# Symb0x76/ChineseChessZero

Measured on NVIDIA B200. Metric: self-play moves/sec at 400 playouts, higher is better.
Workload: dtype bf16

## Files before the change

### chinesechesszero_b200/_lib.py

```python
from __future__ import annotations

import ctypes
import os

import numpy as np
import torch

from . import build as _build

BOARD_BYTES = 96
MAX_MOVES = 128
N_ACTIONS = 2086
PLANE_ELEMS = 10710
KEY_WINDOW = 128

FLAG_CHECK, FLAG_NOMOVES, FLAG_INSUFFICIENT, FLAG_FOURFOLD, FLAG_SIXTY = 1, 2, 4, 8, 16
FLAG_TIE_MASK = FLAG_INSUFFICIENT | FLAG_FOURFOLD | FLAG_SIXTY
STATUS_EXPAND_FAILED, STATUS_TREE_DROPPED = 1, 2
STATUS_NODE_OVERFLOW = STATUS_EXPAND_FAILED
ADVANCE_NEW_GAME, ADVANCE_DROP_TREE, ADVANCE_KEEP = -1, -2, -3
CTL_HEAD, CTL_TAIL, CTL_EXPAND_FAILED, CTL_TREES_DROPPED, CTL_MIN_FREE, CTL_WORDS = 0, 1, 2, 3, 4, 8
NODE_BYTES = 24
MAX_CHILDREN = 119
POLICY_PROBS, POLICY_LOGITS = 0, 1
CONV_VARIANT_1CTA, CONV_VARIANT_PAIR, CONV_VARIANT_2PAIRS, CONV_VARIANT_4PAIRS = 1, 2, 2 | 32, 2 | 64

EXPORTS = (
    "ccz_version", "ccz_last_error", "ccz_init", "ccz_action_table", "ccz_set_order_policy", "ccz_get_order_policy",
    "ccz_boards_start",
    "ccz_movegen_encode", "ccz_board_keys_init", "ccz_board_push", "ccz_mcts_pool_init", "ccz_mcts_reset",
    "ccz_mcts_reserve", "ccz_mcts_migrate", "ccz_mcts_select",
    "ccz_mcts_expand_backup", "ccz_mcts_root_visits", "ccz_mcts_advance", "ccz_replay_pack", "ccz_conv3x3_c256", "ccz_conv3x3_plan", "ccz_stem_lookup",
    "ccz_heads_pack",
)


class CczError(RuntimeError):
    pass


class ArenaStruct(ctypes.Structure):

    _fields_ = [
        ("n_games", ctypes.c_int32),
        ("n_pages", ctypes.c_int32),
        ("page_shift", ctypes.c_int32),
        ("max_pages", ctypes.c_int32),
        ("d_nodes", ctypes.c_void_p),
        ("d_links", ctypes.c_void_p),
        ("d_free_ring", ctypes.c_void_p),
        ("d_pool_ctl", ctypes.c_void_p),
        ("d_page_list", ctypes.c_void_p),
        ("d_page_fill", ctypes.c_void_p),
        ("d_n_pages", ctypes.c_void_p),
        ("d_n_pages_new", ctypes.c_void_p),
        ("d_list_sel", ctypes.c_void_p),
        ("d_alloc_page", ctypes.c_void_p),
        ("d_alloc_off", ctypes.c_void_p),
        ("d_root", ctypes.c_void_p),
        ("d_n_nodes", ctypes.c_void_p),
        ("d_status", ctypes.c_void_p),
        ("d_root_boards", ctypes.c_void_p),
        ("d_root_keys", ctypes.c_void_p),
    ]


_lib = None


def library_path() -> str:
    return os.environ.get("CCZ_LIB") or _build.OUT


def load() -> ctypes.CDLL:
    global _lib
    if _lib is not None:
        return _lib
    path = library_path()
    if path == _build.OUT and _build.is_stale():
        try:
            _build.build()
        except Exception as e:
            if not os.path.exists(path):
                raise CczError(f"building {path} failed ({e}); there is no CPU fallback") from e
    if not os.path.exists(path):
        raise CczError(
            f"{path} is missing: run `python -c 'import __graft_entry__ as g; g.build()'` "
            "(nvcc -gencode arch=compute_100a,code=sm_100a); there is no CPU fallback"
        )
    lib = ctypes.CDLL(path)
    vp, i32, f32 = ctypes.c_void_p, ctypes.c_int, ctypes.c_float
    lib.ccz_version.restype = i32
    lib.ccz_last_error.restype = ctypes.c_char_p
    lib.ccz_init.restype = i32
    lib.ccz_action_table.argtypes = [vp, vp, vp]
    lib.ccz_boards_start.argtypes = [vp, i32, vp]
    lib.ccz_set_order_policy.argtypes = [vp]
    lib.ccz_get_order_policy.argtypes = [vp]
    lib.ccz_movegen_encode.argtypes = [vp, i32, vp, vp, vp, vp, vp]
    lib.ccz_board_keys_init.argtypes = [vp, i32, vp, vp]
    lib.ccz_board_push.argtypes = [vp, vp, i32, vp, vp]
    lib.ccz_mcts_pool_init.argtypes = [ctypes.POINTER(ArenaStruct), vp]
    lib.ccz_mcts_reset.argtypes = [ctypes.POINTER(ArenaStruct), vp, vp]
    lib.ccz_mcts_reserve.argtypes = [ctypes.POINTER(ArenaStruct), i32, vp]
    lib.ccz_mcts_migrate.argtypes = [ctypes.POINTER(ArenaStruct), ctypes.POINTER(ArenaStruct), vp]
    lib.ccz_mcts_select.argtypes = [ctypes.POINTER(ArenaStruct), f32, vp, vp, vp]
    lib.ccz_mcts_expand_backup.argtypes = [ctypes.POINTER(ArenaStruct), vp, vp, i32, vp, vp, vp, vp, vp]
    lib.ccz_mcts_root_visits.argtypes = [ctypes.POINTER(ArenaStruct), vp, vp, vp, vp]
    lib.ccz_mcts_advance.argtypes = [ctypes.POINTER(ArenaStruct), vp, vp]
    lib.ccz_replay_pack.argtypes = [vp, vp, vp, vp, vp, i32, vp, vp, vp]
    lib.ccz_conv3x3_c256.argtypes = [vp, vp, vp, vp, vp, i32, i32, vp]
    lib.ccz_stem_lookup.argtypes = [vp, i32, vp, vp, vp, vp]
    lib.ccz_conv3x3_plan.argtypes = [i32, i32, i32, vp]
    lib.ccz_heads_pack.argtypes = [vp, i32, vp, i32, i32, vp]
    for name in EXPORTS:
        if name not in ("ccz_last_error",):
            getattr(lib, name).restype = i32
    _lib = lib
    pinned = os.path.join(os.path.dirname(os.path.abspath(__file__)), "order_policy.json")
    if os.path.exists(pinned):
        import json

        with open(pinned) as f:
            set_order_policy(json.load(f))
    return lib


def check(rc: int, what: str) -> None:
    if rc != 0:
        msg = load().ccz_last_error().decode("utf-8", "replace")
        raise CczError(f"{what} failed ({rc}): {msg}")


def stream_ptr(device=None) -> int:
    return torch.cuda.current_stream(device).cuda_stream


def _ptr(t: torch.Tensor | None) -> int | None:
    if t is None:
        return None
    if not t.is_cuda:
        raise CczError("device tensor expected (the C ABI takes device pointers)")
    if not t.is_contiguous():
        raise CczError("contiguous tensor expected")
    return t.data_ptr()


def host_action_table():
    id_of = np.empty(8100, dtype=np.int16)
    fr = np.empty(N_ACTIONS, dtype=np.uint8)
    to = np.empty(N_ACTIONS, dtype=np.uint8)
    n = load().ccz_action_table(id_of.ctypes.data, fr.ctypes.data, to.ctypes.data)
    if n != N_ACTIONS:
        raise CczError(f"ccz_action_table returned {n}")
    return id_of.reshape(90, 90), fr, to


PIECE_SYMBOLS = (None, "p", "c", "r", "n", "b", "a", "k")
DEFAULT_ORDER_POLICY = {"class_rank": {"p": 1, "c": 0, "r": 0, "n": 0, "b": 0, "a": 0, "k": 0},
                        "from_descending": 1, "to_descending": 1, "capture_mode": 0, "check_king_first": 0}


def set_order_policy(policy: dict | None = None) -> None:
    if policy is None:
        check(load().ccz_set_order_policy(None), "ccz_set_order_policy")
        return
    ranks = [0] * 8
    for sym, r in policy["class_rank"].items():
        ranks[PIECE_SYMBOLS.index(sym)] = int(r)
    raw = bytes(ranks + [int(policy["from_descending"]), int(policy["to_descending"]), int(policy["capture_mode"]),
                        int(policy.get("check_king_first", 0))])
    check(load().ccz_set_order_policy(ctypes.create_string_buffer(raw, 12)), "ccz_set_order_policy")


def get_order_policy() -> dict:
    buf = ctypes.create_string_buffer(12)
    check(load().ccz_get_order_policy(buf), "ccz_get_order_policy")
    b = buf.raw
    return {"class_rank": {PIECE_SYMBOLS[t]: b[t] for t in range(1, 8)}, "from_descending": b[8],
            "to_descending": b[9], "capture_mode": b[10], "check_king_first": b[11]}



def boards_start(n: int, device="cuda") -> torch.Tensor:
    boards = torch.empty((n, BOARD_BYTES), dtype=torch.uint8, device=device)
    with torch.cuda.device(boards.device):
        check(load().ccz_boards_start(_ptr(boards), n, stream_ptr(boards.device)), "ccz_boards_start")
    return boards


def movegen_encode(boards: torch.Tensor, planes: bool = True, out=None):
    n = boards.shape[0]
    dev = boards.device
    _ptr(boards)
    if out is None:
        move_ids = torch.empty((n, MAX_MOVES), dtype=torch.int16, device=dev)
        counts = torch.empty((n,), dtype=torch.int16, device=dev)
        flags = torch.empty((n,), dtype=torch.uint8, device=dev)
        pl = torch.empty((n, 17, 7, 10, 9), dtype=torch.bfloat16, device=dev) if planes else None
    else:
        move_ids, counts, flags, pl = out
    with torch.cuda.device(dev):
        check(
            load().ccz_movegen_encode(_ptr(boards), n, _ptr(move_ids), _ptr(counts), _ptr(flags), _ptr(pl),
                                      stream_ptr(dev)),
            "ccz_movegen_encode",
        )
    return move_ids, counts, flags, pl


def board_keys_init(boards: torch.Tensor) -> torch.Tensor:
    n = boards.shape[0]
    keys = torch.empty((n, KEY_WINDOW), dtype=torch.int64, device=boards.device)
    with torch.cuda.device(boards.device):
        check(load().ccz_board_keys_init(_ptr(boards), n, _ptr(keys), stream_ptr(boards.device)),
              "ccz_board_keys_init")
    return keys


def board_push(boards: torch.Tensor, move_ids: torch.Tensor, keys: torch.Tensor | None = None) -> None:
    n = boards.shape[0]
    if move_ids.dtype != torch.int16 or move_ids.numel() != n:
        raise CczError("move_ids must be int16 [n]")
    with torch.cuda.device(boards.device):
        check(load().ccz_board_push(_ptr(boards), _ptr(move_ids), n, _ptr(keys), stream_ptr(boards.device)),
              "ccz_board_push")


def search_pages(n_playout: int, page_shift: int) -> int:
    runs_per_page = max(1, (1 << page_shift) // MAX_CHILDREN)
    return -(-int(n_playout) // runs_per_page) + 1


class Arena:

    def __init__(self, n_games: int, n_pages: int, page_shift: int = 11, max_pages: int | None = None, device="cuda"):
        self.n_games, self.n_pages, self.page_shift = int(n_games), int(n_pages), int(page_shift)
        if not 7 <= self.page_shift <= 16:
            raise CczError("page_shift must be 7..16")
        if self.n_pages < self.n_games:
            raise CczError("the pool needs at least one page per game")
        if (self.n_pages << self.page_shift) >= 1 << 31:
            raise CczError("pool too large: n_pages << page_shift must stay below 2^31 nodes")
        self.max_pages = int(max_pages) if max_pages is not None else min(self.n_pages, 4096)
        self.device = torch.device(device)
        total = self.n_pages << self.page_shift
        g, z = self.n_games, dict(device=self.device)
        i32 = torch.int32
        self.nodes = torch.empty((total, 4), dtype=i32, **z)
        self.links = torch.empty((total, 2), dtype=i32, **z)
        self.free_ring = torch.zeros(self.n_pages, dtype=i32, **z)
        self.pool_ctl = torch.zeros(CTL_WORDS, dtype=torch.int64, **z)
        self.page_lists = torch.zeros((2, g, self.max_pages), dtype=i32, **z)
        self.page_fill = torch.zeros((g, self.max_pages), dtype=i32, **z)
        self.n_pages_game = torch.zeros(g, dtype=i32, **z)
        self.n_pages_new = torch.zeros(g, dtype=i32, **z)
        self.list_sel = torch.zeros(g, dtype=i32, **z)
        self.alloc_page = torch.zeros(g, dtype=i32, **z)
        self.alloc_off = torch.zeros(g, dtype=i32, **z)
        self.root = torch.zeros(g, dtype=i32, **z)
        self.n_nodes = torch.zeros(g, dtype=i32, **z)
        self.status = torch.zeros(g, dtype=i32, **z)
        self.root_boards = torch.zeros((g, BOARD_BYTES), dtype=torch.uint8, **z)
        self.root_keys = torch.zeros((g, KEY_WINDOW), dtype=torch.int64, **z)
        self._tensors = (self.nodes, self.links, self.free_ring, self.pool_ctl, self.page_lists, self.page_fill,
                         self.n_pages_game, self.n_pages_new, self.list_sel, self.alloc_page, self.alloc_off, self.root,
                         self.n_nodes, self.status, self.root_boards, self.root_keys)
        self.struct = ArenaStruct(self.n_games, self.n_pages, self.page_shift, self.max_pages,
                                  *(t.data_ptr() for t in self._tensors))
        with torch.cuda.device(self.device):
            check(load().ccz_mcts_pool_init(self.ref, stream_ptr(self.device)), "ccz_mcts_pool_init")

    @property
    def ref(self):
        return ctypes.byref(self.struct)

    @property
    def page_nodes(self) -> int:
        return 1 << self.page_shift

    def bytes(self) -> int:
        return sum(t.numel() * t.element_size() for t in self._tensors)

    def pool_stats(self) -> dict:
        c = self.pool_ctl.cpu().numpy()
        free = int(c[CTL_TAIL] - c[CTL_HEAD])
        return {"n_pages": self.n_pages, "page_nodes": self.page_nodes, "free_pages": free,
                "min_free_pages": int(c[CTL_MIN_FREE]), "expand_failed": int(c[CTL_EXPAND_FAILED]),
                "trees_dropped": int(c[CTL_TREES_DROPPED])}

    def node_fields(self, idx: torch.Tensor) -> dict:
        idx = idx.to(torch.int64)
        n, l = self.nodes[idx], self.links[idx]
        word = l[..., 1]
        return {"visits": n[..., 0], "value": n[..., 1].contiguous().view(torch.float32),
                "prior": n[..., 2].contiguous().view(torch.float32), "first_child": n[..., 3], "parent": l[..., 0],
                "move": ((word & 0xFFFF) ^ 0x8000) - 0x8000, "n_child": word >> 16}

    def children(self, node: int) -> dict:
        f = self.node_fields(torch.tensor([node], device=self.device))
        fc, nc = int(f["first_child"][0]), int(f["n_child"][0])
        return self.node_fields(torch.arange(fc, fc + nc, device=self.device))


def mcts_reset(a: Arena, mask: torch.Tensor | None = None) -> None:
    if mask is not None and (mask.dtype != torch.uint8 or mask.numel() != a.n_games):
        raise CczError("mask must be uint8 [n_games]")
    with torch.cuda.device(a.device):
        check(load().ccz_mcts_reset(a.ref, _ptr(mask), stream_ptr(a.device)), "ccz_mcts_reset")


def mcts_select(a: Arena, c_puct: float, leaf_boards: torch.Tensor, leaf_nodes: torch.Tensor) -> None:
    with torch.cuda.device(a.device):
        check(load().ccz_mcts_select(a.ref, float(c_puct), _ptr(leaf_boards), _ptr(leaf_nodes), stream_ptr(a.device)),
              "ccz_mcts_select")


def mcts_expand_backup(a: Arena, leaf_nodes, policy, policy_kind, values, move_ids, counts, flags) -> None:
    if policy.dtype != torch.float32 or values.dtype != torch.float32:
        raise CczError("policy and values must be float32")
    with torch.cuda.device(a.device):
        check(
            load().ccz_mcts_expand_backup(a.ref, _ptr(leaf_nodes), _ptr(policy), int(policy_kind), _ptr(values),
                                          _ptr(move_ids), _ptr(counts), _ptr(flags), stream_ptr(a.device)),
            "ccz_mcts_expand_backup",
        )


def mcts_root_visits(a: Arena, acts, visits, counts) -> None:
    with torch.cuda.device(a.device):
        check(load().ccz_mcts_root_visits(a.ref, _ptr(acts), _ptr(visits), _ptr(counts), stream_ptr(a.device)),
              "ccz_mcts_root_visits")


def mcts_advance(a: Arena, chosen: torch.Tensor) -> None:
    if chosen.dtype != torch.int16 or chosen.numel() != a.n_games:
        raise CczError("chosen must be int16 [n_games]")
    with torch.cuda.device(a.device):
        check(load().ccz_mcts_advance(a.ref, _ptr(chosen), stream_ptr(a.device)), "ccz_mcts_advance")


def mcts_reserve(a: Arena, pages_per_game: int) -> None:
    with torch.cuda.device(a.device):
        check(load().ccz_mcts_reserve(a.ref, int(pages_per_game), stream_ptr(a.device)), "ccz_mcts_reserve")


def mcts_migrate(src: Arena, dst: Arena) -> None:
    with torch.cuda.device(src.device):
        check(load().ccz_mcts_migrate(src.ref, dst.ref, stream_ptr(src.device)), "ccz_mcts_migrate")


def replay_pack(hist_boards, turn_plane, acts, probs, counts):
    n = hist_boards.shape[0]
    dev = hist_boards.device
    states = torch.empty((2 * n, 17, 7, 10, 9), dtype=torch.float16, device=dev)
    pi = torch.empty((2 * n, N_ACTIONS), dtype=torch.float64, device=dev)
    with torch.cuda.device(dev):
        check(
            load().ccz_replay_pack(_ptr(hist_boards), _ptr(turn_plane), _ptr(acts), _ptr(probs), _ptr(counts), n,
                                   _ptr(states), _ptr(pi), stream_ptr(dev)),
            "ccz_replay_pack",
        )
    return states, pi


def conv3x3_c256(x: torch.Tensor, w: torch.Tensor, bias: torch.Tensor, skip: torch.Tensor | None = None,
                 out: torch.Tensor | None = None, variant: int = 0) -> torch.Tensor:
    cl = torch.channels_last
    if x.dtype != torch.bfloat16 or w.dtype != torch.bfloat16 or bias.dtype != torch.float32:
        raise CczError("conv3x3_c256: x and w must be bfloat16, bias float32")
    if tuple(x.shape[1:]) != (256, 10, 9) or tuple(w.shape) != (256, 256, 3, 3) or bias.numel() != 256:
        raise CczError("conv3x3_c256: shapes must be x (n,256,10,9), w (256,256,3,3), bias (256,)")
    if not x.is_contiguous(memory_format=cl) or not w.is_contiguous(memory_format=cl):
        raise CczError("conv3x3_c256: x and w must be channels_last")
    if skip is not None and (skip.shape != x.shape or skip.dtype != x.dtype or not skip.is_contiguous(memory_format=cl)):
        raise CczError("conv3x3_c256: skip must match x (bf16, channels_last)")
    if out is None:
        out = torch.empty_like(x, memory_format=cl)
    elif out.shape != x.shape or out.dtype != x.dtype or not out.is_contiguous(memory_format=cl):
        raise CczError("conv3x3_c256: out must match x (bf16, channels_last)")
    if not 0 <= variant < 128:
        raise CczError("conv3x3_c256: variant out of range (see ccz_conv3x3_c256 in include/ccz_b200.h)")
    if not (x.is_cuda and w.is_cuda and bias.is_cuda and out.is_cuda):
        raise CczError("device tensor expected (the C ABI takes device pointers)")
    with torch.cuda.device(x.device):
        check(
            load().ccz_conv3x3_c256(x.data_ptr(), w.data_ptr(), bias.data_ptr(), None if skip is None else skip.data_ptr(),
                                    out.data_ptr(), int(x.shape[0]), int(variant), stream_ptr(x.device)),
            "ccz_conv3x3_c256",
        )
    return out


def stem_lookup(boards: torch.Tensor, table: torch.Tensor, bias_turn: torch.Tensor, out: torch.Tensor | None = None) -> torch.Tensor:
    n = boards.shape[0]
    if boards.dtype != torch.uint8 or boards.shape[1:] != (BOARD_BYTES,):
        raise CczError("stem_lookup: boards must be uint8 (n,96)")
    if table.dtype != torch.bfloat16 or tuple(table.shape) != (9, 16, 256) or bias_turn.dtype != torch.float32 \
            or tuple(bias_turn.shape) != (2, 9, 256):
        raise CczError("stem_lookup: table must be bf16 (9,16,256) and bias_turn fp32 (2,9,256)")
    if out is None:
        out = torch.empty((n, 256, 10, 9), dtype=torch.bfloat16, device=boards.device).contiguous(memory_format=torch.channels_last)
    elif tuple(out.shape) != (n, 256, 10, 9) or out.dtype != torch.bfloat16 or not out.is_contiguous(memory_format=torch.channels_last):
        raise CczError("stem_lookup: out must be bf16 (n,256,10,9) channels_last")
    with torch.cuda.device(boards.device):
        check(load().ccz_stem_lookup(_ptr(boards), n, _ptr(table), _ptr(bias_turn), out.data_ptr(), stream_ptr(boards.device)),
              "ccz_stem_lookup")
    return out


def heads_pack(h: torch.Tensor, operands: torch.Tensor, value_off: int) -> torch.Tensor:
    n = operands.shape[0]
    if h.dtype != torch.bfloat16 or operands.dtype != torch.bfloat16 or tuple(h.shape) != (n * 90, 32):
        raise CczError("heads_pack: h must be bf16 (n*90, 32) and operands bf16 (n, K)")
    with torch.cuda.device(h.device):
        check(load().ccz_heads_pack(_ptr(h), n, _ptr(operands), int(operands.shape[1]), int(value_off), stream_ptr(h.device)),
              "ccz_heads_pack")
    return operands


def conv3x3_plan(n_boards: int, variant: int = 0, resident_clusters: int = 74) -> dict:
    out = (ctypes.c_int32 * 6)()
    check(load().ccz_conv3x3_plan(int(n_boards), int(variant), int(resident_clusters), out), "ccz_conv3x3_plan")
    keys = ("rows_per_tile", "n_tiles", "n_items", "n_full", "split_log2", "clusters")
    return dict(zip(keys, (int(v) for v in out)))
```

### chinesechesszero_b200/build.py

```python
from __future__ import annotations

import os
import subprocess

_HERE = os.path.dirname(os.path.abspath(__file__))
CSRC = os.path.join(_HERE, "csrc")
OUT = os.path.join(CSRC, "libccz_b200.so")
SOURCES = ["ccz_b200.cu"]
HEADERS = ["ccz_rules.cuh", "ccz_movegen.cuh", "ccz_mcts.cuh", "ccz_replay.cuh", "ccz_conv.cuh", "ccz_stem.cuh", "ccz_heads.cuh", "../../include/ccz_b200.h"]
NVCC_FLAGS = [
    "-gencode", "arch=compute_100a,code=sm_100a",
    "-lineinfo", "-O3", "-std=c++17",
    "-shared", "-Xcompiler", "-fPIC",
]


def _nvcc() -> str:
    cand = os.path.join(os.environ.get("CUDA_HOME", "/usr/local/cuda"), "bin", "nvcc")
    return cand if os.path.exists(cand) else "nvcc"


def is_stale() -> bool:
    if not os.path.exists(OUT):
        return True
    t = os.path.getmtime(OUT)
    return any(os.path.getmtime(os.path.join(CSRC, f)) > t for f in SOURCES + HEADERS)


def build(force: bool = False, verbose: bool = False) -> str:
    if force or is_stale():
        tmp = OUT + f".tmp{os.getpid()}"
        cmd = [_nvcc(), *NVCC_FLAGS, "-o", tmp, *SOURCES]
        if verbose:
            cmd.insert(1, "-Xptxas")
            cmd.insert(2, "-v")
        subprocess.run(cmd, check=True, cwd=CSRC)
        os.replace(tmp, OUT)
    return OUT


if __name__ == "__main__":
    print(build(force=True, verbose=True))
```

### chinesechesszero_b200/csrc/ccz_b200.cu

```cuda
#include "../../include/ccz_b200.h"

#include <cuda_runtime.h>

#include <cstdio>
#include <cstdlib>
#include <cstring>
#include <utility>
#include <string>

#include "ccz_movegen.cuh"
#include "ccz_mcts.cuh"
#include "ccz_replay.cuh"
#include "ccz_conv.cuh"
#include "ccz_stem.cuh"
#include "ccz_heads.cuh"

#ifndef CCZ_CONV_DEFAULT_PAIRS
#define CCZ_CONV_DEFAULT_PAIRS 1
#endif

namespace {

thread_local std::string g_err;

int fail(int code, const char *what, cudaError_t e = cudaSuccess) {
    g_err = what;
    if (e != cudaSuccess) {
        g_err += ": ";
        g_err += cudaGetErrorString(e);
    }
    return code;
}

#define CCZ_CUDA(call)                                      \
    do {                                                    \
        cudaError_t e_ = (call);                            \
        if (e_ != cudaSuccess) return fail(-2, #call, e_);  \
    } while (0)

struct HostTables {
    int16_t id_of[8100];
    uint8_t from_of[ccz::N_ACTIONS], to_of[ccz::N_ACTIONS];
    int16_t flip_of[ccz::N_ACTIONS];
    uint64_t zkeys[16 * 90 + 1];
    uint8_t start[ccz::BOARD_BYTES];
    uint16_t step_tab[ccz::STEP_TAB_ENTRIES];
    bool built = false;
};
HostTables g_tab;
bool g_dev_ready[64] = {false};
const ccz_order_policy kDefaultPolicy = {{0, 1, 0, 0, 0, 0, 0, 0}, 1, 1, 0, 0};
ccz_order_policy g_policy = kDefaultPolicy;
bool g_policy_is_default = true;
unsigned g_policy_version = 1, g_dev_policy_version[64] = {0};

int sq_of(const char *s) { return (s[0] - 'a') + 9 * (s[1] - '0'); }

void build_step_table(uint16_t *tab) {
    for (int i = 0; i < ccz::STEP_TAB_ENTRIES; ++i) tab[i] = 0xFFFF;
    for (int piece = 0; piece < 5; ++piece)
        for (int black = 0; black < (piece == 4 ? 1 : 2); ++black)
            for (int sq = 0; sq < 90; ++sq) {
                const int r = sq / 9, f = sq % 9;
                int to[8], blk[8], m = 0;
                auto add = [&](int rr, int ff, int b) {
                    if (rr < 0 || rr > 9 || ff < 0 || ff > 8) return;
                    to[m] = rr * 9 + ff;
                    blk[m++] = b;
                };
                auto in_palace = [&](int rr, int ff) {
                    return ff >= 3 && ff <= 5 && (black ? (rr >= 7 && rr <= 9) : (rr >= 0 && rr <= 2));
                };
                if (piece == 0) {
                    add(r + (black ? -1 : 1), f, 127);
                    if (black ? r <= 4 : r >= 5) { add(r, f - 1, 127); add(r, f + 1, 127); }
                } else if (piece == 4) {
                    static const int d[8][2] = {{2, 1}, {2, -1}, {-2, 1}, {-2, -1}, {1, 2}, {1, -2}, {-1, 2}, {-1, -2}};
                    for (auto &k : d) {
                        const int lr = r + (k[0] == 2 ? 1 : k[0] == -2 ? -1 : 0);
                        const int lf = f + (k[1] == 2 ? 1 : k[1] == -2 ? -1 : 0);
                        add(r + k[0], f + k[1], lr * 9 + lf);
                    }
                } else if (piece == 1) {
                    for (int a = -2; a <= 2; a += 4)
                        for (int c = -2; c <= 2; c += 4) {
                            const int rr = r + a;
                            if (rr < 0 || rr > 9 || (black ? rr < 5 : rr > 4)) continue;
                            add(rr, f + c, (r + a / 2) * 9 + f + c / 2);
                        }
                } else if (piece == 2) {
                    for (int a = -1; a <= 1; a += 2)
                        for (int c = -1; c <= 1; c += 2)
                            if (in_palace(r + a, f + c)) add(r + a, f + c, 127);
                } else {
                    static const int d[4][2] = {{1, 0}, {-1, 0}, {0, 1}, {0, -1}};
                    for (auto &k : d)
                        if (in_palace(r + k[0], f + k[1])) add(r + k[0], f + k[1], 127);
                }
                for (int i = 0; i < m; ++i)
                    for (int j = i + 1; j < m; ++j)
                        if (to[j] > to[i]) { std::swap(to[i], to[j]); std::swap(blk[i], blk[j]); }
                uint16_t *e = piece == 4 ? tab + sq * 8
                                         : tab + ccz::STEP_KNIGHT_ENTRIES + ((piece * 2 + black) * 90 + sq) * 4;
                for (int i = 0; i < m; ++i) e[i] = (uint16_t)(to[i] | (blk[i] << 7));
            }
}

void build_tables() {
    if (g_tab.built) return;
    HostTables &t = g_tab;
    for (int i = 0; i < 8100; ++i) t.id_of[i] = -1;
    int idx = 0;
    auto add = [&](int from, int to) {
        t.id_of[from * 90 + to] = (int16_t)idx;
        t.from_of[idx] = (uint8_t)from;
        t.to_of[idx] = (uint8_t)to;
        ++idx;
    };
    static const int kn[8][2] = {{-2, -1}, {-1, -2}, {-2, 1}, {1, -2}, {2, -1}, {-1, 2}, {2, 1}, {1, 2}};
    for (int rank = 0; rank < 10; ++rank)
        for (int file = 0; file < 9; ++file) {
            const int from = file + 9 * rank;
            for (int r2 = 0; r2 < 10; ++r2)
                if (r2 != rank) add(from, file + 9 * r2);
            for (int f2 = 0; f2 < 9; ++f2)
                if (f2 != file) add(from, f2 + 9 * rank);
            for (auto &k : kn) {
                const int r2 = rank + k[0], f2 = file + k[1];
                if (r2 >= 0 && r2 < 10 && f2 >= 0 && f2 < 9) add(from, f2 + 9 * r2);
            }
        }
    static const char *const advisor[] = {"d0e1", "e1d0", "f0e1", "e1f0", "d2e1", "e1d2", "f2e1", "e1f2",
                                          "d9e8", "e8d9", "f9e8", "e8f9", "d7e8", "e8d7", "f7e8", "e8f7"};
    static const char *const elephant[] = {
        "a2c0", "c0a2", "a2c4", "c4a2", "c0e2", "e2c0", "c4e2", "e2c4", "e2g0", "g0e2", "e2g4",
        "g4e2", "g0i2", "i2g0", "g4i2", "i2g4", "a7c5", "c5a7", "a7c9", "c9a7", "c5e7", "e7c5",
        "c9e7", "e7c9", "e7g5", "g5e7", "e7g9", "g9e7", "g5i7", "i7g5", "g9i7", "i7g9"};
    for (const char *m : advisor) add(sq_of(m), sq_of(m + 2));
    for (const char *m : elephant) add(sq_of(m), sq_of(m + 2));
    for (int i = 0; i < ccz::N_ACTIONS; ++i) {
        const int f = t.from_of[i], to = t.to_of[i];
        const int mf = (8 - f % 9) + 9 * (f / 9), mt = (8 - to % 9) + 9 * (to / 9);
        t.flip_of[i] = t.id_of[mf * 90 + mt];
    }
    uint64_t x = 0x0123456789ABCDEFull;
    for (int i = 0; i < 16 * 90 + 1; ++i) {
        x += 0x9E3779B97F4A7C15ull;
        uint64_t z = x;
        z = (z ^ (z >> 30)) * 0xBF58476D1CE4E5B9ull;
        z = (z ^ (z >> 27)) * 0x94D049BB133111EBull;
        t.zkeys[i] = z ^ (z >> 31);
    }
    std::memset(t.start, 0, sizeof(t.start));
    static const uint8_t back[9] = {3, 4, 5, 6, 7, 6, 5, 4, 3};
    for (int f = 0; f < 9; ++f) {
        t.start[f] = back[f];
        t.start[81 + f] = back[f] | 8;
    }
    t.start[19] = t.start[25] = 2;
    t.start[64] = t.start[70] = 2 | 8;
    for (int f = 0; f < 9; f += 2) {
        t.start[27 + f] = 1;
        t.start[54 + f] = 1 | 8;
    }
    t.start[ccz::OFF_TURN] = 1;
    build_step_table(t.step_tab);
    t.built = (idx == ccz::N_ACTIONS);
}

int ensure_device() {
    build_tables();
    if (!g_tab.built) return fail(-3, "action table construction failed");
    int dev = 0;
    CCZ_CUDA(cudaGetDevice(&dev));
    if (dev < 0 || dev >= 64) return fail(-3, "device index out of range");
    if (g_dev_policy_version[dev] != g_policy_version) {
        CCZ_CUDA(cudaMemcpyToSymbol(ccz::d_order_policy, &g_policy, sizeof(g_policy)));
        g_dev_policy_version[dev] = g_policy_version;
    }
    if (g_dev_ready[dev]) return 0;
    CCZ_CUDA(cudaMemcpyToSymbol(ccz::d_id_of, g_tab.id_of, sizeof(g_tab.id_of)));
    CCZ_CUDA(cudaMemcpyToSymbol(ccz::d_from_of, g_tab.from_of, sizeof(g_tab.from_of)));
    CCZ_CUDA(cudaMemcpyToSymbol(ccz::d_to_of, g_tab.to_of, sizeof(g_tab.to_of)));
    CCZ_CUDA(cudaMemcpyToSymbol(ccz::d_flip_of, g_tab.flip_of, sizeof(g_tab.flip_of)));
    CCZ_CUDA(cudaMemcpyToSymbol(ccz::d_zkeys, g_tab.zkeys, sizeof(g_tab.zkeys)));
    CCZ_CUDA(cudaMemcpyToSymbol(ccz::d_start_board, g_tab.start, sizeof(g_tab.start)));
    CCZ_CUDA(cudaMemcpyToSymbol(ccz::d_step_tab, g_tab.step_tab, sizeof(g_tab.step_tab)));
    g_dev_ready[dev] = true;
    return 0;
}

int sm_count() {
    static int cached = 0;
    if (!cached) {
        int dev = 0;
        cudaGetDevice(&dev);
        cudaDeviceGetAttribute(&cached, cudaDevAttrMultiProcessorCount, dev);
        if (cached <= 0) cached = 148;
    }
    return cached;
}

int check_launch(const char *what) {
    cudaError_t e = cudaGetLastError();
    if (e != cudaSuccess) return fail(-2, what, e);
    return 0;
}

int check_arena(const ccz_arena *a) {
    if (!a) return fail(-1, "arena is NULL");
    if (a->n_games <= 0 || a->n_pages < a->n_games || a->max_pages < 1) return fail(-1, "arena geometry invalid");
    if (a->page_shift < 7 || a->page_shift > 16 || ((long long)a->n_pages << a->page_shift) > 0x7fffffffll)
        return fail(-1, "arena geometry invalid: page_shift must be 7..16 and n_pages << page_shift < 2^31");
    if (!a->d_nodes || !a->d_links || !a->d_free_ring || !a->d_pool_ctl || !a->d_page_list || !a->d_page_fill ||
        !a->d_n_pages || !a->d_n_pages_new || !a->d_list_sel || !a->d_alloc_page || !a->d_alloc_off || !a->d_root ||
        !a->d_n_nodes || !a->d_status || !a->d_root_boards || !a->d_root_keys)
        return fail(-1, "arena has a NULL array");
    if (((uintptr_t)a->d_nodes & 15) || ((uintptr_t)a->d_links & 7) || ((uintptr_t)a->d_pool_ctl & 7))
        return fail(-1, "arena node arrays must be 16-byte aligned");
    return 0;
}

inline int warps_grid(int n) { return (n + ccz::MCTS_WARPS - 1) / ccz::MCTS_WARPS; }

}

extern "C" {

int ccz_version(void) { return 200; }

const char *ccz_last_error(void) { return g_err.c_str(); }

int ccz_init(void) { return ensure_device(); }

int ccz_action_table(int16_t *id_of, uint8_t *from_of, uint8_t *to_of) {
    build_tables();
    if (!g_tab.built) return fail(-3, "action table construction failed");
    if (id_of) std::memcpy(id_of, g_tab.id_of, sizeof(g_tab.id_of));
    if (from_of) std::memcpy(from_of, g_tab.from_of, sizeof(g_tab.from_of));
    if (to_of) std::memcpy(to_of, g_tab.to_of, sizeof(g_tab.to_of));
    return ccz::N_ACTIONS;
}

int ccz_set_order_policy(const ccz_order_policy *p) {
    static_assert(sizeof(ccz_order_policy) == 12, "ccz_order_policy layout");
    const ccz_order_policy &q = p ? *p : kDefaultPolicy;
    if (q.capture_mode > 2 || q.from_descending > 1 || q.to_descending > 1 || q.check_king_first > 1)
        return fail(-1, "ccz_set_order_policy: from_descending / to_descending / check_king_first must be 0|1, capture_mode 0|1|2");
    for (int t = 1; t <= 7; ++t)
        if (q.class_rank[t] > 7) return fail(-1, "ccz_set_order_policy: class_rank must be 0..7");
    g_policy = q;
    g_policy.class_rank[0] = 0;
    g_policy_is_default = std::memcmp(&g_policy, &kDefaultPolicy, sizeof(g_policy)) == 0;
    ++g_policy_version;
    return 0;
}

int ccz_get_order_policy(ccz_order_policy *out) {
    if (!out) return fail(-1, "ccz_get_order_policy: NULL");
    *out = g_policy;
    return 0;
}

int ccz_boards_start(uint8_t *d_boards, int n, ccz_stream_t s) {
    if (n < 0 || (n > 0 && !d_boards)) return fail(-1, "ccz_boards_start: bad arguments");
    if (int rc = ensure_device()) return rc;
    if (n == 0) return 0;
    const int threads = 256, total = n * 6;
    ccz::boards_start_kernel<<<(total + threads - 1) / threads, threads, 0, s>>>(d_boards, n);
    return check_launch("boards_start_kernel");
}

int ccz_movegen_encode(const uint8_t *d_boards, int n, int16_t *d_move_ids, int16_t *d_counts, uint8_t *d_flags,
                       void *d_planes_bf16, ccz_stream_t s) {
    if (n < 0) return fail(-1, "ccz_movegen_encode: n < 0");
    if (n == 0) return 0;
    if (!d_boards || !d_move_ids || !d_counts || !d_flags) return fail(-1, "ccz_movegen_encode: NULL pointer");
    if (((uintptr_t)d_boards & 15) || ((uintptr_t)d_move_ids & 7) || ((uintptr_t)d_planes_bf16 & 15))
        return fail(-1, "ccz_movegen_encode: boards/planes must be 16-byte, move_ids 8-byte aligned");
    if (int rc = ensure_device()) return rc;
    const int n_quads = (n + 3) / 4;
    int grid = (n_quads + ccz::MG_WARPS - 1) / ccz::MG_WARPS;
    const int cap = sm_count() * CCZ_MG_MIN_BLOCKS;
    if (grid > cap) grid = cap;
    static unsigned int *claim_base[64] = {nullptr};
    static unsigned launch_no = 0;
    int dev = 0;
    CCZ_CUDA(cudaGetDevice(&dev));
    if (!claim_base[dev]) {
        cudaFuncSetAttribute(ccz::movegen_encode_kernel<false>, cudaFuncAttributePreferredSharedMemoryCarveout, 100);
        cudaFuncSetAttribute(ccz::movegen_encode_kernel<true>, cudaFuncAttributePreferredSharedMemoryCarveout, 100);
        CCZ_CUDA(cudaGetSymbolAddress(reinterpret_cast<void **>(&claim_base[dev]), ccz::d_mg_counter));
    }
    unsigned int *claim = claim_base[dev] + (launch_no++ % ccz::MG_COUNTER_SLOTS);
    CCZ_CUDA(cudaMemsetAsync(claim, 0, sizeof(unsigned int), s));
    if (g_policy_is_default)
        ccz::movegen_encode_kernel<false><<<grid, ccz::MG_WARPS * 32, 0, s>>>(d_boards, n, d_move_ids, d_counts, d_flags,
                                                                             static_cast<uint32_t *>(d_planes_bf16), claim);
    else
        ccz::movegen_encode_kernel<true><<<grid, ccz::MG_WARPS * 32, 0, s>>>(d_boards, n, d_move_ids, d_counts, d_flags,
                                                                            static_cast<uint32_t *>(d_planes_bf16), claim);
    return check_launch("movegen_encode_kernel");
}

int ccz_board_keys_init(const uint8_t *d_boards, int n, uint64_t *d_keys, ccz_stream_t s) {
    if (n < 0 || (n > 0 && (!d_boards || !d_keys))) return fail(-1, "ccz_board_keys_init: bad arguments");
    if (int rc = ensure_device()) return rc;
    if (n == 0) return 0;
    CCZ_CUDA(cudaMemsetAsync(d_keys, 0xFF, (size_t)n * ccz::KEY_WINDOW * sizeof(uint64_t), s));
    ccz::board_keys_init_kernel<<<warps_grid(n), ccz::MCTS_WARPS * 32, 0, s>>>(d_boards, n, d_keys);
    return check_launch("board_keys_init_kernel");
}

int ccz_board_push(uint8_t *d_boards, const int16_t *d_move_ids, int n, uint64_t *d_keys, ccz_stream_t s) {
    if (n < 0 || (n > 0 && (!d_boards || !d_move_ids))) return fail(-1, "ccz_board_push: bad arguments");
    if (int rc = ensure_device()) return rc;
    if (n == 0) return 0;
    ccz::board_push_kernel<<<warps_grid(n), ccz::MCTS_WARPS * 32, 0, s>>>(d_boards, d_move_ids, n, d_keys);
    return check_launch("board_push_kernel");
}

int ccz_mcts_pool_init(const ccz_arena *a, ccz_stream_t s) {
    if (int rc = check_arena(a)) return rc;
    if (int rc = ensure_device()) return rc;
    const int n_free = a->n_pages - a->n_games;
    int blocks = (n_free + 255) / 256;
    if (blocks < 1) blocks = 1;
    if (blocks > 1024) blocks = 1024;
    ccz::mcts_pool_init_kernel<<<blocks, 256, 0, s>>>(*a);
    if (int rc = check_launch("mcts_pool_init_kernel")) return rc;
    ccz::mcts_games_init_kernel<<<warps_grid(a->n_games), ccz::MCTS_WARPS * 32, 0, s>>>(*a);
    return check_launch("mcts_games_init_kernel");
}

int ccz_mcts_reset(const ccz_arena *a, const uint8_t *d_mask, ccz_stream_t s) {
    if (int rc = check_arena(a)) return rc;
    if (int rc = ensure_device()) return rc;
    ccz::mcts_reset_kernel<<<warps_grid(a->n_games), ccz::MCTS_WARPS * 32, 0, s>>>(*a, d_mask);
    return check_launch("mcts_reset_kernel");
}

int ccz_mcts_reserve(const ccz_arena *a, int pages_per_game, ccz_stream_t s) {
    if (int rc = check_arena(a)) return rc;
    if (pages_per_game < 1) return fail(-1, "ccz_mcts_reserve: pages_per_game < 1");
    if ((long long)a->n_games * (pages_per_game + 1) > a->n_pages || pages_per_game + 1 > a->max_pages)
        return fail(-1, "ccz_mcts_reserve: the pool cannot hold pages_per_game + 1 pages for every game");
    if (int rc = ensure_device()) return rc;
    ccz::mcts_reserve_kernel<<<warps_grid(a->n_games), ccz::MCTS_WARPS * 32, 0, s>>>(*a, pages_per_game);
    return check_launch("mcts_reserve_kernel");
}

int ccz_mcts_migrate(const ccz_arena *src, const ccz_arena *dst, ccz_stream_t s) {
    if (int rc = check_arena(src)) return rc;
    if (int rc = check_arena(dst)) return rc;
    if (src->n_games != dst->n_games) return fail(-1, "ccz_mcts_migrate: n_games differs");
    if (src->d_nodes == dst->d_nodes || src->d_pool_ctl == dst->d_pool_ctl)
        return fail(-1, "ccz_mcts_migrate: src and dst must be distinct arenas");
    if (int rc = ensure_device()) return rc;
    ccz::mcts_migrate_kernel<<<warps_grid(src->n_games), ccz::MCTS_WARPS * 32, 0, s>>>(*src, *dst);
    return check_launch("mcts_migrate_kernel");
}

int ccz_mcts_select(const ccz_arena *a, float c_puct, uint8_t *d_leaf_boards, int32_t *d_leaf_nodes,
                    ccz_stream_t s) {
    if (int rc = check_arena(a)) return rc;
    if (!d_leaf_boards || !d_leaf_nodes) return fail(-1, "ccz_mcts_select: NULL output");
    if (int rc = ensure_device()) return rc;
    static const bool staged = [] { const char *e = std::getenv("CCZ_SELECT_STAGED"); return !(e && e[0] == '0'); }();
    if (staged)
        ccz::mcts_select_kernel<true><<<warps_grid(a->n_games), ccz::MCTS_WARPS * 32, 0, s>>>(*a, c_puct, d_leaf_boards,
                                                                                             d_leaf_nodes);
    else
        ccz::mcts_select_kernel<false><<<warps_grid(a->n_games), ccz::MCTS_WARPS * 32, 0, s>>>(*a, c_puct, d_leaf_boards,
                                                                                              d_leaf_nodes);
    return check_launch("mcts_select_kernel");
}

int ccz_mcts_expand_backup(const ccz_arena *a, const int32_t *d_leaf_nodes, const float *d_policy, int policy_kind,
                           const float *d_values, const int16_t *d_move_ids, const int16_t *d_counts,
                           const uint8_t *d_flags, ccz_stream_t s) {
    if (int rc = check_arena(a)) return rc;
    if (!d_leaf_nodes || !d_policy || !d_values || !d_move_ids || !d_counts || !d_flags)
        return fail(-1, "ccz_mcts_expand_backup: NULL pointer");
    if (policy_kind != CCZ_POLICY_PROBS && policy_kind != CCZ_POLICY_LOGITS)
        return fail(-1, "ccz_mcts_expand_backup: unknown policy_kind");
    if (int rc = ensure_device()) return rc;
    ccz::mcts_expand_backup_kernel<<<warps_grid(a->n_games), ccz::MCTS_WARPS * 32, 0, s>>>(
        *a, d_leaf_nodes, d_policy, policy_kind, d_values, d_move_ids, d_counts, d_flags);
    return check_launch("mcts_expand_backup_kernel");
}

int ccz_mcts_root_visits(const ccz_arena *a, int16_t *d_acts, int32_t *d_visits, int16_t *d_counts,
                         ccz_stream_t s) {
    if (int rc = check_arena(a)) return rc;
    if (!d_acts || !d_visits || !d_counts) return fail(-1, "ccz_mcts_root_visits: NULL output");
    if (int rc = ensure_device()) return rc;
    ccz::mcts_root_visits_kernel<<<warps_grid(a->n_games), ccz::MCTS_WARPS * 32, 0, s>>>(*a, d_acts, d_visits,
                                                                                        d_counts);
    return check_launch("mcts_root_visits_kernel");
}

int ccz_mcts_advance(const ccz_arena *a, const int16_t *d_chosen, ccz_stream_t s) {
    if (int rc = check_arena(a)) return rc;
    if (!d_chosen) return fail(-1, "ccz_mcts_advance: NULL chosen");
    if (int rc = ensure_device()) return rc;
    ccz::mcts_advance_compact_kernel<<<warps_grid(a->n_games), ccz::MCTS_WARPS * 32, 0, s>>>(*a, d_chosen);
    if (int rc = check_launch("mcts_advance_compact_kernel")) return rc;
    ccz::mcts_advance_release_kernel<<<warps_grid(a->n_games), ccz::MCTS_WARPS * 32, 0, s>>>(*a);
    return check_launch("mcts_advance_release_kernel");
}

int ccz_replay_pack(const uint8_t *d_hist_boards, const uint8_t *d_turn_plane, const int16_t *d_acts,
                    const double *d_probs, const int16_t *d_counts, int n, void *d_states_f16, double *d_pi,
                    ccz_stream_t s) {
    if (n < 0) return fail(-1, "ccz_replay_pack: n < 0");
    if (n == 0) return 0;
    if (!d_hist_boards || !d_turn_plane || !d_acts || !d_probs || !d_counts || !d_states_f16 || !d_pi)
        return fail(-1, "ccz_replay_pack: NULL pointer");
    if (int rc = ensure_device()) return rc;
    const long long words = 2ll * n * ccz::WORDS_PER_POS;
    const int threads = 256;
    const long long blocks = (words + threads - 1) / threads;
    if (blocks > 0x7fffffffll) return fail(-1, "ccz_replay_pack: n too large");
    ccz::replay_states_kernel<<<(unsigned)blocks, threads, 0, s>>>(d_hist_boards, d_turn_plane, n,
                                                                   static_cast<uint32_t *>(d_states_f16));
    if (int rc = check_launch("replay_states_kernel")) return rc;
    CCZ_CUDA(cudaMemsetAsync(d_pi, 0, (size_t)2 * n * ccz::N_ACTIONS * sizeof(double), s));
    ccz::replay_pi_kernel<<<(n * 32 + threads - 1) / threads, threads, 0, s>>>(d_acts, d_probs, d_counts, n, d_pi);
    return check_launch("replay_pi_kernel");
}

int ccz_conv3x3_c256(const void *d_x, const void *d_w, const float *d_bias, const void *d_skip, void *d_y, int n_boards,
                     int variant, ccz_stream_t s) {
    namespace cv = ccz::conv;
    if (n_boards < 0) return fail(-1, "ccz_conv3x3_c256: n_boards < 0");
    if (n_boards == 0) return 0;
    if (!d_x || !d_w || !d_bias || !d_y) return fail(-1, "ccz_conv3x3_c256: NULL pointer");
    if (d_y == d_x) return fail(-1, "ccz_conv3x3_c256: output must not alias the input (halo reads)");
    if (variant < 0 || variant >= 128) return fail(-1, "ccz_conv3x3_c256: bad variant");
    int cta_group = variant & 3;
    const int tail_split = !(variant & 4), dbg = (variant >> 3) & 3;
    int pairs = 1 << ((variant >> 5) & 3);
#ifndef CCZ_CONV_EXPERIMENTS
    if (dbg) return fail(-1, "ccz_conv3x3_c256: the load-skipping measurement variants need a -DCCZ_CONV_EXPERIMENTS build");
#endif
    if (variant == 0) { cta_group = 2; pairs = CCZ_CONV_DEFAULT_PAIRS; }
    if (cta_group == 0) cta_group = 2;
    if (cta_group == 3 || pairs > 4 || (cta_group == 1 && pairs != 1))
        return fail(-1, "ccz_conv3x3_c256: unsupported variant (cta_group 1|2, pairs 1|2|4, pairs > 1 needs cta_group 2)");
    if (((uintptr_t)d_x | (uintptr_t)d_w | (uintptr_t)d_y | (uintptr_t)d_skip) & 15)
        return fail(-1, "ccz_conv3x3_c256: pointers must be 16-byte aligned");
    static cv::Driver drv;
    if (const char *err = cv::driver_init(drv)) return fail(-3, err);
    const long long m = (long long)n_boards * cv::BOARD_HW;
    const int rows_per_tile = cv::BM * cta_group * pairs;
    const int n_tiles = (int)((m + rows_per_tile - 1) / rows_per_tile);
    CUtensorMap tx, tw, ts, ty;
    if (!cv::encode_im2col(drv, &tx, d_x, n_boards)) return fail(-3, "ccz_conv3x3_c256: cuTensorMapEncodeIm2col(x) failed");
    if (!cv::encode_rows(drv, &tw, d_w, cv::BN, 9 * cv::C, (uint32_t)(cv::BN / cta_group / pairs)))
        return fail(-3, "ccz_conv3x3_c256: cuTensorMapEncodeTiled(w) failed");
    if (!cv::encode_rows(drv, &ty, d_y, (uint64_t)m, cv::C, cv::BM)) return fail(-3, "ccz_conv3x3_c256: cuTensorMapEncodeTiled(y) failed");
    if (d_skip) {
        if (!cv::encode_rows(drv, &ts, d_skip, (uint64_t)m, cv::C, cv::BM))
            return fail(-3, "ccz_conv3x3_c256: cuTensorMapEncodeTiled(skip) failed");
    } else {
        ts = ty;
    }
    cudaError_t e;
#define CCZ_CONV_LAUNCH(CG, PAIRS)                                                                                      \
    (d_skip ? cv::launch_variant<CG, PAIRS, true>(tx, tw, ts, ty, d_bias, n_tiles, tail_split, dbg, s)     \
            : cv::launch_variant<CG, PAIRS, false>(tx, tw, ts, ty, d_bias, n_tiles, tail_split, dbg, s))
    if (cta_group == 1) e = CCZ_CONV_LAUNCH(1, 1);
    else if (pairs == 1) e = CCZ_CONV_LAUNCH(2, 1);
    else if (pairs == 2) e = CCZ_CONV_LAUNCH(2, 2);
    else e = CCZ_CONV_LAUNCH(2, 4);
#undef CCZ_CONV_LAUNCH
    if (e != cudaSuccess) return fail(-2, "conv3x3_c256_kernel launch", e);
    return 0;
}

int ccz_conv3x3_plan(int n_boards, int variant, int resident_clusters, int32_t *out) {
    namespace cv = ccz::conv;
    if (n_boards <= 0 || resident_clusters <= 0 || !out || variant < 0 || variant >= 128)
        return fail(-1, "ccz_conv3x3_plan: bad argument");
    int cta_group = variant & 3, pairs = 1 << ((variant >> 5) & 3);
    if (variant == 0) { cta_group = 2; pairs = CCZ_CONV_DEFAULT_PAIRS; }
    if (cta_group == 0) cta_group = 2;
    if (cta_group == 3 || pairs > 4 || (cta_group == 1 && pairs != 1)) return fail(-1, "ccz_conv3x3_plan: unsupported variant");
    const long long m = (long long)n_boards * cv::BOARD_HW;
    const int rows_per_tile = cv::BM * cta_group * pairs;
    const int n_tiles = (int)((m + rows_per_tile - 1) / rows_per_tile);
    const cv::Plan pl = cv::plan_items(n_tiles, resident_clusters, !(variant & 4));
    out[0] = rows_per_tile; out[1] = n_tiles; out[2] = pl.n_items; out[3] = pl.n_full; out[4] = pl.split_log2; out[5] = pl.clusters;
    return 0;
}

int ccz_stem_lookup(const uint8_t *d_boards, int n, const void *d_table, const float *d_bias_turn, void *d_y, ccz_stream_t s) {
    namespace st = ccz::stem;
    if (n < 0) return fail(-1, "ccz_stem_lookup: n < 0");
    if (n == 0) return 0;
    if (!d_boards || !d_table || !d_bias_turn || !d_y) return fail(-1, "ccz_stem_lookup: NULL pointer");
    if (((uintptr_t)d_boards & 3) || (((uintptr_t)d_table | (uintptr_t)d_bias_turn | (uintptr_t)d_y) & 15))
        return fail(-1, "ccz_stem_lookup: pointers must be 16-byte aligned (boards 4-byte)");
    static int n_sm_dev[64] = {0};
    int dev = 0;
    CCZ_CUDA(cudaGetDevice(&dev));
    if (dev < 0 || dev >= 64) return fail(-1, "ccz_stem_lookup: device index out of range");
    int &n_sm = n_sm_dev[dev];
    if (!n_sm) {
        CCZ_CUDA(cudaDeviceGetAttribute(&n_sm, cudaDevAttrMultiProcessorCount, dev));
        CCZ_CUDA(cudaFuncSetAttribute(st::stem_lookup_kernel, cudaFuncAttributeMaxDynamicSharedMemorySize, st::SMEM_BYTES));
    }
    int blocks = 2 * n_sm;
    const int need = (n + st::WARPS - 1) / st::WARPS;
    if (blocks > need) blocks = need;
    st::stem_lookup_kernel<<<blocks, st::WARPS * 32, st::SMEM_BYTES, s>>>(d_boards, n, static_cast<const uint4 *>(d_table),
                                                                         reinterpret_cast<const float4 *>(d_bias_turn),
                                                                         static_cast<uint4 *>(d_y));
    return check_launch("stem_lookup_kernel");
}

int ccz_heads_pack(const void *d_h, int n, void *d_operands, int row_elems, int value_off, ccz_stream_t s) {
    namespace hd = ccz::heads;
    if (n < 0) return fail(-1, "ccz_heads_pack: n < 0");
    if (n == 0) return 0;
    if (!d_h || !d_operands) return fail(-1, "ccz_heads_pack: NULL pointer");
    if (((uintptr_t)d_h & 15) || ((uintptr_t)d_operands & 3)) return fail(-1, "ccz_heads_pack: h must be 16-byte, operands 4-byte aligned");
    if ((row_elems & 1) || (value_off & 1) || value_off < hd::N_POLICY * hd::HW || row_elems < value_off + hd::N_VALUE * hd::HW)
        return fail(-1, "ccz_heads_pack: operand row must hold 1530 policy + 630 value elements at even offsets");
    hd::heads_pack_kernel<<<n, hd::THREADS, 0, s>>>(static_cast<const uint4 *>(d_h), static_cast<uint32_t *>(d_operands), n,
                                                  row_elems / 2, value_off / 2);
    return check_launch("heads_pack_kernel");
}

}
```

### chinesechesszero_b200/csrc/ccz_conv.cuh

```cuda
#pragma once

#include <cuda.h>
#include <cuda_bf16.h>
#include <cuda_runtime.h>

#include <cstdint>

#ifndef CCZ_CONV_BACKOFF_NS
#define CCZ_CONV_BACKOFF_NS 256
#endif

namespace ccz {
namespace conv {

constexpr int C = 256;
constexpr int BOARD_H = 10, BOARD_W = 9, BOARD_HW = 90;
constexpr int BM = 128;
constexpr int BN = 256;
constexpr int BK = 64;
constexpr int KBLOCKS = 9 * (C / BK);
constexpr int UMMA_K = 16;
constexpr int THREADS = 256;

template <int CG>
struct Cfg {
    static constexpr int B_ROWS = BN / CG;
    static constexpr int A_BYTES = BM * BK * 2;
    static constexpr int B_BYTES = B_ROWS * BK * 2;
    static constexpr int STAGE_BYTES = A_BYTES + B_BYTES;
    static constexpr int STAGES = CG == 2 ? 5 : 3;
    static constexpr int STAGING_BYTES = BM * BN * 2;
    static constexpr int BIAS_BYTES = BN * 4;
    static constexpr int BAR_BYTES = 256;
    static constexpr int SMEM_BYTES = 1024  + STAGES * STAGE_BYTES + STAGING_BYTES + BIAS_BYTES + BAR_BYTES;
};

__device__ __forceinline__ uint32_t smem_u32(const void *p) { return (uint32_t)__cvta_generic_to_shared(p); }

__device__ __forceinline__ uint32_t cluster_ctarank() {
    uint32_t r;
    asm volatile("mov.u32 %0, %%cluster_ctarank;" : "=r"(r));
    return r;
}
__device__ __forceinline__ uint32_t mapa(uint32_t addr, uint32_t rank) {
    uint32_t r;
    asm volatile("mapa.shared::cluster.u32 %0, %1, %2;" : "=r"(r) : "r"(addr), "r"(rank));
    return r;
}
__device__ __forceinline__ void mbar_init(uint32_t bar, uint32_t count) {
    asm volatile("mbarrier.init.shared::cta.b64 [%0], %1;" ::"r"(bar), "r"(count) : "memory");
}
__device__ __forceinline__ void mbar_expect_tx(uint32_t bar, uint32_t bytes) {
    asm volatile("mbarrier.arrive.expect_tx.shared::cta.b64 _, [%0], %1;" ::"r"(bar), "r"(bytes) : "memory");
}
__device__ __forceinline__ void mbar_arrive(uint32_t bar) {
    asm volatile("mbarrier.arrive.shared::cta.b64 _, [%0];" ::"r"(bar) : "memory");
}
__device__ __forceinline__ void mbar_arrive_cluster(uint32_t cluster_bar) {
    asm volatile("mbarrier.arrive.release.cluster.shared::cluster.b64 _, [%0];" ::"r"(cluster_bar) : "memory");
}
__device__ __forceinline__ void mbar_wait(uint32_t bar, uint32_t parity) {
    asm volatile(
        "{\n"
        ".reg .pred P1;\n"
        "LAB_WAIT:\n"
        "mbarrier.try_wait.parity.shared::cta.b64 P1, [%0], %1;\n"
        "@P1 bra DONE;\n"
        "bra LAB_WAIT;\n"
        "DONE:\n"
        "}" ::"r"(bar),
        "r"(parity)
        : "memory");
}
__device__ __forceinline__ void mbar_wait_relaxed(uint32_t bar, uint32_t parity) {
    for (;;) {
        uint32_t done;
        asm volatile(
            "{\n"
            ".reg .pred P1;\n"
            "mbarrier.try_wait.parity.shared::cta.b64 P1, [%1], %2;\n"
            "selp.u32 %0, 1, 0, P1;\n"
            "}"
            : "=r"(done)
            : "r"(bar), "r"(parity)
            : "memory");
        if (done) break;
        __nanosleep(CCZ_CONV_BACKOFF_NS);
    }
}
__device__ __forceinline__ void mbar_wait_cluster(uint32_t bar, uint32_t parity) {
    asm volatile(
        "{\n"
        ".reg .pred P1;\n"
        "LAB_WAIT:\n"
        "mbarrier.try_wait.parity.acquire.cluster.shared::cta.b64 P1, [%0], %1;\n"
        "@P1 bra DONE;\n"
        "bra LAB_WAIT;\n"
        "DONE:\n"
        "}" ::"r"(bar),
        "r"(parity)
        : "memory");
}
__device__ __forceinline__ void tma_prefetch_desc(const CUtensorMap *m) {
    asm volatile("prefetch.tensormap [%0];" ::"l"(reinterpret_cast<uint64_t>(m)) : "memory");
}

constexpr uint64_t L2_HINT_DEFAULT = 0x1000000000000000ull;

template <int CG>
__device__ __forceinline__ void tma_load_2d(uint32_t dst, const CUtensorMap *m, uint32_t bar, int c0, int c1) {
    if constexpr (CG == 1) {
        asm volatile("cp.async.bulk.tensor.2d.shared::cluster.global.mbarrier::complete_tx::bytes [%0], [%1, {%3, %4}], [%2];" ::"r"(dst),
                     "l"(reinterpret_cast<uint64_t>(m)), "r"(bar), "r"(c0), "r"(c1)
                     : "memory");
    } else {
        asm volatile(
            "cp.async.bulk.tensor.2d.cta_group::2.shared::cluster.global.mbarrier::complete_tx::bytes.L2::cache_hint [%0], [%1, {%3, %4}], "
            "[%2], %5;" ::"r"(dst),
            "l"(reinterpret_cast<uint64_t>(m)), "r"(bar), "r"(c0), "r"(c1), "l"(L2_HINT_DEFAULT)
            : "memory");
    }
}
template <int CG>
__device__ __forceinline__ void tma_load_im2col(uint32_t dst, const CUtensorMap *m, uint32_t bar, int c, int w, int h, int n, uint16_t off_w,
                                                uint16_t off_h) {
    if constexpr (CG == 1) {
        asm volatile(
            "cp.async.bulk.tensor.4d.shared::cluster.global.im2col.mbarrier::complete_tx::bytes [%0], [%1, {%3, %4, %5, %6}], [%2], {%7, %8};" ::
                "r"(dst),
            "l"(reinterpret_cast<uint64_t>(m)), "r"(bar), "r"(c), "r"(w), "r"(h), "r"(n), "h"(off_w), "h"(off_h)
            : "memory");
    } else {
        asm volatile(
            "cp.async.bulk.tensor.4d.im2col.cta_group::2.shared::cluster.global.mbarrier::complete_tx::bytes.L2::cache_hint [%0], [%1, {%3, %4, "
            "%5, %6}], [%2], {%7, %8}, %9;" ::"r"(dst),
            "l"(reinterpret_cast<uint64_t>(m)), "r"(bar), "r"(c), "r"(w), "r"(h), "r"(n), "h"(off_w), "h"(off_h), "l"(L2_HINT_DEFAULT)
            : "memory");
    }
}
__device__ __forceinline__ void tma_store_2d(const CUtensorMap *m, uint32_t src, int c0, int c1) {
    asm volatile("cp.async.bulk.tensor.2d.global.shared::cta.bulk_group [%0, {%2, %3}], [%1];" ::"l"(reinterpret_cast<uint64_t>(m)), "r"(src),
                 "r"(c0), "r"(c1)
                 : "memory");
}
__device__ __forceinline__ void tma_store_commit() { asm volatile("cp.async.bulk.commit_group;" ::: "memory"); }
__device__ __forceinline__ void tma_store_wait_read() { asm volatile("cp.async.bulk.wait_group.read 0;" ::: "memory"); }
__device__ __forceinline__ void tma_store_wait_all() { asm volatile("cp.async.bulk.wait_group 0;" ::: "memory"); }
__device__ __forceinline__ void fence_proxy_async() { asm volatile("fence.proxy.async.shared::cta;" ::: "memory"); }

__device__ __forceinline__ void tc_fence_before() { asm volatile("tcgen05.fence::before_thread_sync;" ::: "memory"); }
__device__ __forceinline__ void tc_fence_after() { asm volatile("tcgen05.fence::after_thread_sync;" ::: "memory"); }

template <int CG>
__device__ __forceinline__ void tmem_alloc(uint32_t slot_smem, uint32_t cols) {
    if constexpr (CG == 1) {
        asm volatile("tcgen05.alloc.cta_group::1.sync.aligned.shared::cta.b32 [%0], %1;" ::"r"(slot_smem), "r"(cols) : "memory");
        asm volatile("tcgen05.relinquish_alloc_permit.cta_group::1.sync.aligned;" ::: "memory");
    } else {
        asm volatile("tcgen05.alloc.cta_group::2.sync.aligned.shared::cta.b32 [%0], %1;" ::"r"(slot_smem), "r"(cols) : "memory");
        asm volatile("tcgen05.relinquish_alloc_permit.cta_group::2.sync.aligned;" ::: "memory");
    }
}
template <int CG>
__device__ __forceinline__ void tmem_dealloc(uint32_t taddr, uint32_t cols) {
    if constexpr (CG == 1)
        asm volatile("tcgen05.dealloc.cta_group::1.sync.aligned.b32 %0, %1;" ::"r"(taddr), "r"(cols) : "memory");
    else
        asm volatile("tcgen05.dealloc.cta_group::2.sync.aligned.b32 %0, %1;" ::"r"(taddr), "r"(cols) : "memory");
}
template <int CG>
__device__ __forceinline__ void umma_bf16(uint32_t d_tmem, uint64_t a_desc, uint64_t b_desc, uint32_t idesc, uint32_t accumulate) {
    if constexpr (CG == 1) {
        asm volatile(
            "{\n.reg .pred p;\nsetp.ne.b32 p, %4, 0;\n"
            "tcgen05.mma.cta_group::1.kind::f16 [%0], %1, %2, %3, p;\n}" ::"r"(d_tmem),
            "l"(a_desc), "l"(b_desc), "r"(idesc), "r"(accumulate)
            : "memory");
    } else {
        asm volatile(
            "{\n.reg .pred p;\nsetp.ne.b32 p, %4, 0;\n"
            "tcgen05.mma.cta_group::2.kind::f16 [%0], %1, %2, %3, p;\n}" ::"r"(d_tmem),
            "l"(a_desc), "l"(b_desc), "r"(idesc), "r"(accumulate)
            : "memory");
    }
}
template <int CG>
__device__ __forceinline__ void umma_commit(uint32_t bar, uint16_t cta_mask) {
    if constexpr (CG == 1) {
        asm volatile("tcgen05.commit.cta_group::1.mbarrier::arrive::one.shared::cluster.b64 [%0];" ::"r"(bar) : "memory");
    } else {
        asm volatile("tcgen05.commit.cta_group::2.mbarrier::arrive::one.shared::cluster.multicast::cluster.b64 [%0], %1;" ::"r"(bar),
                     "h"(cta_mask)
                     : "memory");
    }
}
__device__ __forceinline__ void tma_load_2d_mc(uint32_t dst, const CUtensorMap *m, uint32_t bar, int c0, int c1, uint16_t cta_mask) {
    asm volatile(
        "cp.async.bulk.tensor.2d.cta_group::2.shared::cluster.global.mbarrier::complete_tx::bytes.multicast::cluster.L2::cache_hint [%0], [%1, "
        "{%4, %5}], [%2], %3, %6;" ::"r"(dst),
        "l"(reinterpret_cast<uint64_t>(m)), "r"(bar), "h"(cta_mask), "r"(c0), "r"(c1), "l"(L2_HINT_DEFAULT)
        : "memory");
}
__device__ __forceinline__ void tmem_ld32(uint32_t taddr, uint32_t (&v)[32]) {
    asm volatile(
        "tcgen05.ld.sync.aligned.32x32b.x32.b32 "
        "{%0, %1, %2, %3, %4, %5, %6, %7, %8, %9, %10, %11, %12, %13, %14, %15, "
        "%16, %17, %18, %19, %20, %21, %22, %23, %24, %25, %26, %27, %28, %29, %30, %31}, [%32];"
        : "=r"(v[0]), "=r"(v[1]), "=r"(v[2]), "=r"(v[3]), "=r"(v[4]), "=r"(v[5]), "=r"(v[6]), "=r"(v[7]), "=r"(v[8]), "=r"(v[9]),
          "=r"(v[10]), "=r"(v[11]), "=r"(v[12]), "=r"(v[13]), "=r"(v[14]), "=r"(v[15]), "=r"(v[16]), "=r"(v[17]), "=r"(v[18]),
          "=r"(v[19]), "=r"(v[20]), "=r"(v[21]), "=r"(v[22]), "=r"(v[23]), "=r"(v[24]), "=r"(v[25]), "=r"(v[26]), "=r"(v[27]),
          "=r"(v[28]), "=r"(v[29]), "=r"(v[30]), "=r"(v[31])
        : "r"(taddr)
        : "memory");
}
__device__ __forceinline__ void tmem_ld_wait() { asm volatile("tcgen05.wait::ld.sync.aligned;" ::: "memory"); }

__device__ __forceinline__ void cluster_sync_all() {
    asm volatile("barrier.cluster.arrive.release.aligned;\nbarrier.cluster.wait.acquire.aligned;" ::: "memory");
}

__device__ __forceinline__ uint64_t umma_desc_sw128(uint32_t smem_addr) {
    return (uint64_t)((smem_addr >> 4) & 0x3FFF) | (1ull << 16) | (64ull << 32) | (1ull << 46) | (2ull << 61);
}
__host__ __device__ constexpr uint32_t umma_idesc(int m, int n) {
    return (1u << 4) | (1u << 7) | (1u << 10) | ((uint32_t)(n >> 3) << 17) | ((uint32_t)(m >> 4) << 24);
}

__device__ __forceinline__ uint32_t pack_bf16x2(float lo, float hi) {
    __nv_bfloat162 t = __floats2bfloat162_rn(lo, hi);
    return *reinterpret_cast<uint32_t *>(&t);
}

struct WorkItem {
    int tile, n_off, n_w;
};
__device__ __forceinline__ WorkItem work_item(int i, int n_full, int split_log2) {
    if (i < n_full) return {i, 0, BN};
    const int j = i - n_full, n_w = BN >> split_log2;
    return {n_full + (j >> split_log2), (j & ((1 << split_log2) - 1)) * n_w, n_w};
}

template <int CG, int PAIRS, bool HAS_SKIP>
__global__ void __launch_bounds__(THREADS, 1)
conv3x3_c256_kernel(const __grid_constant__ CUtensorMap tm_x, const __grid_constant__ CUtensorMap tm_w,
                    const __grid_constant__ CUtensorMap tm_skip, const __grid_constant__ CUtensorMap tm_y, const float *__restrict__ bias,
                    int n_items, int n_full, int split_log2, int dbg) {
    using K = Cfg<CG>;
    extern __shared__ uint8_t smem_raw[];
    const uint32_t smem_base = (smem_u32(smem_raw) + 1023u) & ~1023u;
    const uint32_t a_smem = smem_base;
    const uint32_t b_smem = a_smem + K::STAGES * K::A_BYTES;
    const uint32_t staging = b_smem + K::STAGES * K::B_BYTES;
    const uint32_t bias_smem = staging + K::STAGING_BYTES;
    const uint32_t bars = bias_smem + K::BIAS_BYTES;
    const uint32_t bar_full = bars;
    const uint32_t bar_empty = bars + 8 * K::STAGES;
    const uint32_t bar_tfull = bars + 16 * K::STAGES;
    const uint32_t bar_tempty = bar_tfull + 16;
    const uint32_t bar_skip = bar_tempty + 16;
    const uint32_t bar_stfree = bar_skip + 8;
    const uint32_t tmem_slot = bar_stfree + 8;
    uint8_t *const smem_gen = smem_raw + (smem_base - smem_u32(smem_raw));

    const int warp = threadIdx.x >> 5, lane = threadIdx.x & 31;
    static_assert(CG == 2 || PAIRS == 1, "weight multicast needs CTA pairs");
    constexpr int CLUSTER = CG * PAIRS;
    const uint32_t rank = CLUSTER > 1 ? cluster_ctarank() : 0u;
    const uint32_t prank = rank % CG, pair_id = rank / CG, lead_rank = rank - prank;
    const int cluster_id = blockIdx.x / CLUSTER, n_clusters = gridDim.x / CLUSTER;

    if (warp == 0 && lane == 0) {
        tma_prefetch_desc(&tm_x);
        tma_prefetch_desc(&tm_w);
        tma_prefetch_desc(&tm_y);
        if (HAS_SKIP) tma_prefetch_desc(&tm_skip);
    }
    if (warp == 1 && lane == 0) {
        for (int i = 0; i < K::STAGES; ++i) {
            mbar_init(bar_full + 8 * i, 1);
            mbar_init(bar_empty + 8 * i, PAIRS);
        }
        for (int i = 0; i < 2; ++i) {
            mbar_init(bar_tfull + 8 * i, 1);
            mbar_init(bar_tempty + 8 * i, 4 * CG);
        }
        mbar_init(bar_skip, 1);
        mbar_init(bar_stfree, 1);
        asm volatile("fence.mbarrier_init.release.cluster;" ::: "memory");
    }
    if (warp == 2) tmem_alloc<CG>(tmem_slot, 512);
    if (warp >= 4) {
        const int t = threadIdx.x - 128;
        reinterpret_cast<float *>(smem_gen + (bias_smem - smem_base))[t] = bias[t];
        reinterpret_cast<float *>(smem_gen + (bias_smem - smem_base))[t + 128] = bias[t + 128];
    }
    tc_fence_before();
    if constexpr (CLUSTER > 1) cluster_sync_all(); else __syncthreads();
    tc_fence_after();
    const uint32_t tmem_base = *reinterpret_cast<volatile uint32_t *>(smem_gen + (tmem_slot - smem_base));

    if (warp == 0) {
        if (lane == 0) {
            const uint32_t full0 = CG == 2 ? mapa(bar_full, lead_rank) : bar_full;
            constexpr int SLICE_ROWS = K::B_ROWS / PAIRS;
            uint16_t mc_mask = 0;
            for (int j = 0; j < PAIRS; ++j) mc_mask |= (uint16_t)(1u << (j * CG + prank));
            int stage = 0;
            uint32_t phase = 0;
            for (int item = cluster_id; item < n_items; item += n_clusters) {
                const WorkItem wi = work_item(item, n_full, split_log2);
                const int m0 = ((wi.tile * PAIRS + (int)pair_id) * CG + (int)prank) * BM;
                const int b_row = wi.n_off + (int)prank * (wi.n_w / CG);
                const int img = m0 / BOARD_HW, rem = m0 - img * BOARD_HW;
                const int p = rem / BOARD_W, q = rem - p * BOARD_W;
                for (int kb = 0; kb < KBLOCKS; ++kb) {
                    const int tap = kb >> 2, c0 = (kb & 3) * BK;
                    const int r = tap / 3, s = tap - 3 * r;
                    mbar_wait(bar_empty + 8 * stage, phase ^ 1);
                    const bool do_a = !((dbg & 2) && (kb & 1)), do_b = !((dbg & 1) && (kb & 1));
                    if (prank == 0) mbar_expect_tx(bar_full + 8 * stage, CG * ((do_a ? K::A_BYTES : 0) + (do_b ? K::B_BYTES : 0)));
                    if (do_a) tma_load_im2col<CG>(a_smem + stage * K::A_BYTES, &tm_x, full0 + 8 * stage, c0, q - 1, p - 1, img, (uint16_t)s, (uint16_t)r);
                    if constexpr (PAIRS == 1) {
                        if (do_b) tma_load_2d<CG>(b_smem + stage * K::B_BYTES, &tm_w, full0 + 8 * stage, kb * BK, b_row);
                    } else {
                        tma_load_2d_mc(b_smem + stage * K::B_BYTES + (int)pair_id * SLICE_ROWS * 128, &tm_w, full0 + 8 * stage, kb * BK,
                                       b_row + (int)pair_id * SLICE_ROWS, mc_mask);
                    }
                    if (++stage == K::STAGES) { stage = 0; phase ^= 1; }
                }
            }
        }
    } else if (warp == 1) {
        if (prank == 0 && lane == 0) {
            constexpr uint16_t mask_cluster = (uint16_t)((1u << CLUSTER) - 1);
            const uint16_t mask_pair = (uint16_t)(((1u << CG) - 1) << lead_rank);
            int stage = 0;
            uint32_t phase = 0, acc = 0, acc_phase = 0;
            for (int item = cluster_id; item < n_items; item += n_clusters) {
                const uint32_t idesc = umma_idesc(BM * CG, work_item(item, n_full, split_log2).n_w);
                mbar_wait_cluster(bar_tempty + 8 * acc, acc_phase ^ 1);
                tc_fence_after();
                const uint32_t d_tmem = tmem_base + acc * BN;
                for (int kb = 0; kb < KBLOCKS; ++kb) {
                    mbar_wait(bar_full + 8 * stage, phase);
                    tc_fence_after();
                    const uint64_t a_desc = umma_desc_sw128(a_smem + stage * K::A_BYTES);
                    const uint64_t b_desc = umma_desc_sw128(b_smem + stage * K::B_BYTES);
#pragma unroll
                    for (int k = 0; k < BK / UMMA_K; ++k)
                        umma_bf16<CG>(d_tmem, a_desc + 2 * k, b_desc + 2 * k, idesc, (uint32_t)((kb | k) != 0));
                    umma_commit<CG>(bar_empty + 8 * stage, mask_cluster);
                    if (++stage == K::STAGES) { stage = 0; phase ^= 1; }
                }
                umma_commit<CG>(bar_tfull + 8 * acc, mask_pair);
                if (++acc == 2) { acc = 0; acc_phase ^= 1; }
            }
        }
    } else if (warp == 3) {
        if (HAS_SKIP && lane == 0) {
            uint32_t it = 0;
            for (int item = cluster_id; item < n_items; item += n_clusters, ++it) {
                const WorkItem wi = work_item(item, n_full, split_log2);
                const int m0 = ((wi.tile * PAIRS + (int)pair_id) * CG + (int)prank) * BM;
                mbar_wait_relaxed(bar_stfree, (it & 1) ^ 1);
                mbar_expect_tx(bar_skip, (wi.n_w / 64) * (BM * 128));
                for (int g = 0; g < wi.n_w / 64; ++g) tma_load_2d<1>(staging + g * (BM * 128), &tm_skip, bar_skip, wi.n_off + g * 64, m0);
            }
        }
    } else if (warp >= 4) {
        const int quarter = warp - 4, row = quarter * 32 + lane;
        const uint32_t tempty0 = CG == 2 ? mapa(bar_tempty, lead_rank) : bar_tempty;
        const float *bias_s = reinterpret_cast<const float *>(smem_gen + (bias_smem - smem_base));
        uint8_t *stg = smem_gen + (staging - smem_base);
        uint32_t acc = 0, acc_phase = 0, it = 0;
        for (int item = cluster_id; item < n_items; item += n_clusters, ++it) {
            const WorkItem wi = work_item(item, n_full, split_log2);
            const int m0 = ((wi.tile * PAIRS + (int)pair_id) * CG + (int)prank) * BM;
            if (HAS_SKIP) mbar_wait_relaxed(bar_skip, it & 1);
            mbar_wait_relaxed(bar_tfull + 8 * acc, acc_phase);
            tc_fence_after();
            const uint32_t t_row = tmem_base + ((uint32_t)(quarter * 32) << 16) + acc * BN;
#pragma unroll 1
            for (int chunk = 0; chunk < wi.n_w / 32; ++chunk) {
                uint32_t v[32];
                tmem_ld32(t_row + chunk * 32, v);
                tmem_ld_wait();
                uint8_t *box_row = stg + (chunk >> 1) * (BM * 128) + row * 128;
#pragma unroll
                for (int j = 0; j < 4; ++j) {
                    const int c16 = (chunk & 1) * 4 + j;
                    uint4 *cell = reinterpret_cast<uint4 *>(box_row + ((c16 ^ (row & 7)) << 4));
                    const float4 b0 = *reinterpret_cast<const float4 *>(bias_s + wi.n_off + chunk * 32 + j * 8);
                    const float4 b1 = *reinterpret_cast<const float4 *>(bias_s + wi.n_off + chunk * 32 + j * 8 + 4);
                    float f[8] = {__uint_as_float(v[j * 8 + 0]) + b0.x, __uint_as_float(v[j * 8 + 1]) + b0.y,
                                  __uint_as_float(v[j * 8 + 2]) + b0.z, __uint_as_float(v[j * 8 + 3]) + b0.w,
                                  __uint_as_float(v[j * 8 + 4]) + b1.x, __uint_as_float(v[j * 8 + 5]) + b1.y,
                                  __uint_as_float(v[j * 8 + 6]) + b1.z, __uint_as_float(v[j * 8 + 7]) + b1.w};
                    if (HAS_SKIP) {
                        const uint4 sk = *cell;
                        const uint32_t w[4] = {sk.x, sk.y, sk.z, sk.w};
#pragma unroll
                        for (int e = 0; e < 4; ++e) {
                            f[2 * e] += __uint_as_float(w[e] << 16);
                            f[2 * e + 1] += __uint_as_float(w[e] & 0xFFFF0000u);
                        }
                    }
                    uint4 o;
                    o.x = pack_bf16x2(fmaxf(f[0], 0.f), fmaxf(f[1], 0.f));
                    o.y = pack_bf16x2(fmaxf(f[2], 0.f), fmaxf(f[3], 0.f));
                    o.z = pack_bf16x2(fmaxf(f[4], 0.f), fmaxf(f[5], 0.f));
                    o.w = pack_bf16x2(fmaxf(f[6], 0.f), fmaxf(f[7], 0.f));
                    *cell = o;
                }
            }
            tc_fence_before();
            __syncwarp();
            if (lane == 0) {
                if constexpr (CG == 2) mbar_arrive_cluster(tempty0 + 8 * acc); else mbar_arrive(bar_tempty + 8 * acc);
            }
            if (++acc == 2) { acc = 0; acc_phase ^= 1; }
            fence_proxy_async();
            asm volatile("bar.sync 1, 128;" ::: "memory");
            if (threadIdx.x == 128) {
                for (int g = 0; g < wi.n_w / 64; ++g) tma_store_2d(&tm_y, staging + g * (BM * 128), wi.n_off + g * 64, m0);
                tma_store_commit();
                tma_store_wait_read();
                if (HAS_SKIP) mbar_arrive(bar_stfree);
            }
            asm volatile("bar.sync 1, 128;" ::: "memory");
        }
        if (threadIdx.x == 128) tma_store_wait_all();
    }

    __syncwarp();
    tc_fence_before();
    if constexpr (CLUSTER > 1) cluster_sync_all(); else __syncthreads();
    if (warp == 2) {
        tc_fence_after();
        tmem_dealloc<CG>(tmem_base, 512);
    }
}

typedef CUresult (*EncodeTiledFn)(CUtensorMap *, CUtensorMapDataType, cuuint32_t, void *, const cuuint64_t *, const cuuint64_t *,
                                  const cuuint32_t *, const cuuint32_t *, CUtensorMapInterleave, CUtensorMapSwizzle, CUtensorMapL2promotion,
                                  CUtensorMapFloatOOBfill);
typedef CUresult (*EncodeIm2colFn)(CUtensorMap *, CUtensorMapDataType, cuuint32_t, void *, const cuuint64_t *, const cuuint64_t *, const int *,
                                   const int *, cuuint32_t, cuuint32_t, const cuuint32_t *, CUtensorMapInterleave, CUtensorMapSwizzle,
                                   CUtensorMapL2promotion, CUtensorMapFloatOOBfill);

struct Driver {
    EncodeTiledFn tiled = nullptr;
    EncodeIm2colFn im2col = nullptr;
    bool ready = false;
};

inline const char *driver_init(Driver &d) {
    if (d.ready) return nullptr;
    cudaDriverEntryPointQueryResult q;
    void *f = nullptr;
    if (cudaGetDriverEntryPoint("cuTensorMapEncodeTiled", &f, cudaEnableDefault, &q) != cudaSuccess || q != cudaDriverEntryPointSuccess || !f)
        return "cuTensorMapEncodeTiled not available from the driver";
    d.tiled = reinterpret_cast<EncodeTiledFn>(f);
    f = nullptr;
    if (cudaGetDriverEntryPoint("cuTensorMapEncodeIm2col", &f, cudaEnableDefault, &q) != cudaSuccess || q != cudaDriverEntryPointSuccess || !f)
        return "cuTensorMapEncodeIm2col not available from the driver";
    d.im2col = reinterpret_cast<EncodeIm2colFn>(f);
    d.ready = true;
    return nullptr;
}

inline bool encode_rows(const Driver &d, CUtensorMap *m, const void *ptr, uint64_t rows, uint64_t cols, uint32_t box_rows) {
    const cuuint64_t dims[2] = {cols, rows};
    const cuuint64_t strides[1] = {cols * 2};
    const cuuint32_t box[2] = {64, box_rows};
    const cuuint32_t es[2] = {1, 1};
    return d.tiled(m, CU_TENSOR_MAP_DATA_TYPE_BFLOAT16, 2, const_cast<void *>(ptr), dims, strides, box, es, CU_TENSOR_MAP_INTERLEAVE_NONE,
                   CU_TENSOR_MAP_SWIZZLE_128B, CU_TENSOR_MAP_L2_PROMOTION_L2_256B, CU_TENSOR_MAP_FLOAT_OOB_FILL_NONE) == CUDA_SUCCESS;
}

inline bool encode_im2col(const Driver &d, CUtensorMap *m, const void *ptr, int n) {
    const cuuint64_t dims[4] = {(cuuint64_t)C, (cuuint64_t)BOARD_W, (cuuint64_t)BOARD_H, (cuuint64_t)n};
    const cuuint64_t strides[3] = {(cuuint64_t)C * 2, (cuuint64_t)C * 2 * BOARD_W, (cuuint64_t)C * 2 * BOARD_HW};
    const int lower[2] = {-1, -1}, upper[2] = {-1, -1};
    const cuuint32_t es[4] = {1, 1, 1, 1};
    return d.im2col(m, CU_TENSOR_MAP_DATA_TYPE_BFLOAT16, 4, const_cast<void *>(ptr), dims, strides, lower, upper, BK, BM, es,
                    CU_TENSOR_MAP_INTERLEAVE_NONE, CU_TENSOR_MAP_SWIZZLE_128B, CU_TENSOR_MAP_L2_PROMOTION_L2_256B,
                    CU_TENSOR_MAP_FLOAT_OOB_FILL_NONE) == CUDA_SUCCESS;
}

struct Plan {
    int n_items, n_full, split_log2, clusters;
};
inline Plan plan_items(int n_tiles, int clusters, bool tail_split) {
    const int rem = n_tiles % clusters;
    int split_log2 = 0;
    if (tail_split && rem > 0) {
        while (split_log2 < 2 && (rem << (split_log2 + 1)) <= clusters) ++split_log2;
    }
    Plan p;
    p.split_log2 = split_log2;
    p.n_full = split_log2 ? n_tiles - rem : n_tiles;
    p.n_items = p.n_full + (split_log2 ? rem << split_log2 : 0);
    p.clusters = clusters > p.n_items ? p.n_items : clusters;
    return p;
}

template <int CG, int PAIRS, bool HAS_SKIP>
inline cudaError_t launch_variant(const CUtensorMap &tx, const CUtensorMap &tw, const CUtensorMap &ts, const CUtensorMap &ty, const float *bias,
                                  int n_tiles, int tail_split, int dbg, cudaStream_t stream) {
    auto kern = conv3x3_c256_kernel<CG, PAIRS, HAS_SKIP>;
    constexpr int CLUSTER = CG * PAIRS;
    static int max_clusters_dev[64] = {0};
    int dev = 0, n_sm = 0;
    cudaError_t e0 = cudaGetDevice(&dev);
    if (e0 != cudaSuccess) return e0;
    if (dev < 0 || dev >= 64) return cudaErrorInvalidDevice;
    int &max_clusters = max_clusters_dev[dev];
    cudaLaunchConfig_t cfg = {};
    cfg.blockDim = dim3(THREADS);
    cfg.dynamicSmemBytes = Cfg<CG>::SMEM_BYTES;
    cfg.stream = stream;
    cudaLaunchAttribute at[1];
    at[0].id = cudaLaunchAttributeClusterDimension;
    at[0].val.clusterDim.x = CLUSTER;
    at[0].val.clusterDim.y = 1;
    at[0].val.clusterDim.z = 1;
    cfg.attrs = at;
    cfg.numAttrs = 1;
    if (!max_clusters) {
        cudaError_t e = cudaDeviceGetAttribute(&n_sm, cudaDevAttrMultiProcessorCount, dev);
        if (e != cudaSuccess) return e;
        e = cudaFuncSetAttribute(kern, cudaFuncAttributeMaxDynamicSharedMemorySize, Cfg<CG>::SMEM_BYTES);
        if (e != cudaSuccess) return e;
        cfg.gridDim = dim3((unsigned)(n_sm / CLUSTER * CLUSTER));
        int n = 0;
        e = cudaOccupancyMaxActiveClusters(&n, kern, &cfg);
        if (e != cudaSuccess) return e;
        if (n < 1) return cudaErrorInvalidConfiguration;
        max_clusters = n < n_sm / CLUSTER ? n : n_sm / CLUSTER;
    }
    const Plan pl = plan_items(n_tiles, max_clusters, tail_split != 0);
    cfg.gridDim = dim3((unsigned)(pl.clusters * CLUSTER));
    return cudaLaunchKernelEx(&cfg, kern, tx, tw, ts, ty, bias, pl.n_items, pl.n_full, pl.split_log2, dbg);
}

}
}
```

### chinesechesszero_b200/csrc/ccz_heads.cuh

```cuda
#pragma once
#include <cuda_bf16.h>
#include <stdint.h>

namespace ccz {
namespace heads {

constexpr int HW = 90, CH = 32, N_POLICY = 17, N_VALUE = 7, THREADS = 128;

__global__ void __launch_bounds__(THREADS)
heads_pack_kernel(const uint4 *__restrict__ h , uint32_t *__restrict__ out , int n,
                  int row_words, int value_word_off) {
    __shared__ __align__(16) uint16_t s_t[HW][CH + 2];
    const int b = blockIdx.x;
    if (b >= n) return;
    const uint4 *src = h + (size_t)b * (HW * CH * 2 / 16);
    for (int i = threadIdx.x; i < HW * CH * 2 / 16; i += THREADS) {
        const uint4 v = src[i];
        const int row = i >> 2, col = (i & 3) * 8;
        uint32_t *d = reinterpret_cast<uint32_t *>(&s_t[row][col]);
        d[0] = v.x; d[1] = v.y; d[2] = v.z; d[3] = v.w;
    }
    __syncthreads();
    auto relu = [](uint16_t x) -> uint32_t { return (x & 0x8000u) ? 0u : (uint32_t)x; };
    uint32_t *row = out + (size_t)b * row_words;
    for (int w = threadIdx.x; w < N_POLICY * HW / 2; w += THREADS) {
        const int e0 = 2 * w, e1 = e0 + 1;
        row[w] = relu(s_t[e0 % HW][e0 / HW]) | relu(s_t[e1 % HW][e1 / HW]) << 16;
    }
    for (int w = threadIdx.x; w < N_VALUE * HW / 2; w += THREADS) {
        const int e0 = 2 * w, e1 = e0 + 1;
        row[value_word_off + w] = relu(s_t[e0 % HW][N_POLICY + e0 / HW]) | relu(s_t[e1 % HW][N_POLICY + e1 / HW]) << 16;
    }
}

}
}
```

### chinesechesszero_b200/csrc/ccz_stem.cuh

```cuda
#pragma once

#include <cuda_bf16.h>
#include <cuda_runtime.h>

#include <cstdint>

namespace ccz {
namespace stem {

constexpr int C_OUT = 256;
constexpr int TABLE_ELEMS = 9 * 16 * C_OUT;
constexpr int BIAS_TURN_ELEMS = 2 * 9 * C_OUT;
constexpr int WARPS = 16;
constexpr int SMEM_BYTES = TABLE_ELEMS * 2 + BIAS_TURN_ELEMS * 4 + WARPS * 96;

__device__ __forceinline__ void add_row(float (&acc)[8], const uint4 t) {
    const uint32_t v[4] = {t.x, t.y, t.z, t.w};
#pragma unroll
    for (int e = 0; e < 4; ++e) {
        acc[2 * e] += __uint_as_float(v[e] << 16);
        acc[2 * e + 1] += __uint_as_float(v[e] & 0xFFFF0000u);
    }
}

__global__ void __launch_bounds__(WARPS * 32, 2)
stem_lookup_kernel(const uint8_t *__restrict__ boards, int n, const uint4 *__restrict__ table, const float4 *__restrict__ bias_turn,
                   uint4 *__restrict__ y) {
    extern __shared__ __align__(16) uint8_t smem[];
    uint4 *tab_s = reinterpret_cast<uint4 *>(smem);
    float4 *bt_s = reinterpret_cast<float4 *>(smem + TABLE_ELEMS * 2);
    uint8_t *brd_s = smem + TABLE_ELEMS * 2 + BIAS_TURN_ELEMS * 4;
    for (int i = threadIdx.x; i < TABLE_ELEMS * 2 / 16; i += blockDim.x) tab_s[i] = table[i];
    for (int i = threadIdx.x; i < BIAS_TURN_ELEMS * 4 / 16; i += blockDim.x) bt_s[i] = bias_turn[i];
    __syncthreads();

    const int warp = threadIdx.x >> 5, lane = threadIdx.x & 31;
    uint8_t *my_board = brd_s + warp * 96;
    const uint4 *tab_lane = tab_s + lane;
    for (int b = blockIdx.x * WARPS + warp; b < n; b += gridDim.x * WARPS) {
        __syncwarp();
        reinterpret_cast<uint32_t *>(my_board)[lane < 24 ? lane : 0] =
            reinterpret_cast<const uint32_t *>(boards + (size_t)b * 96)[lane < 24 ? lane : 0];
        __syncwarp();
        const int turn = my_board[90] ? 1 : 0;
        uint4 *out = y + (size_t)b * 90 * (C_OUT / 8) + lane;
#pragma unroll 1
        for (int h = 0; h < 10; ++h) {
            const int rc = h == 0 ? 0 : (h == 9 ? 2 : 1);
            uint64_t code[3];
#pragma unroll
            for (int r = 0; r < 3; ++r) {
                const int nh = h + r - 1;
                uint64_t packed = 0;
                if (nh >= 0 && nh <= 9) {
#pragma unroll
                    for (int w = 0; w < 9; ++w) {
                        const uint32_t c = my_board[nh * 9 + w];
                        packed |= (uint64_t)((c & 7) ? (c & 15) : 0) << (4 * w);
                    }
                }
                code[r] = packed;
            }
            const float4 *bt_row = bt_s + ((turn * 9 + rc * 3) * C_OUT + lane * 8) / 4;
#pragma unroll
            for (int w = 0; w < 9; ++w) {
                const int cc = w == 0 ? 0 : (w == 8 ? 2 : 1);
                const float4 a0 = bt_row[cc * (C_OUT / 4)], a1 = bt_row[cc * (C_OUT / 4) + 1];
                float acc[8] = {a0.x, a0.y, a0.z, a0.w, a1.x, a1.y, a1.z, a1.w};
#pragma unroll
                for (int r = 0; r < 3; ++r) {
#pragma unroll
                    for (int s = 0; s < 3; ++s) {
                        const int nw = w + s - 1;
                        if (nw < 0 || nw > 8) continue;
                        const int c = (int)(code[r] >> (4 * nw)) & 15;
                        if (c) add_row(acc, tab_lane[((r * 3 + s) * 16 + c) * (C_OUT / 8)]);
                    }
                }
                uint4 o;
                __nv_bfloat162 p0 = __floats2bfloat162_rn(fmaxf(acc[0], 0.f), fmaxf(acc[1], 0.f));
                __nv_bfloat162 p1 = __floats2bfloat162_rn(fmaxf(acc[2], 0.f), fmaxf(acc[3], 0.f));
                __nv_bfloat162 p2 = __floats2bfloat162_rn(fmaxf(acc[4], 0.f), fmaxf(acc[5], 0.f));
                __nv_bfloat162 p3 = __floats2bfloat162_rn(fmaxf(acc[6], 0.f), fmaxf(acc[7], 0.f));
                o.x = *reinterpret_cast<uint32_t *>(&p0);
                o.y = *reinterpret_cast<uint32_t *>(&p1);
                o.z = *reinterpret_cast<uint32_t *>(&p2);
                o.w = *reinterpret_cast<uint32_t *>(&p3);
                out[(h * 9 + w) * (C_OUT / 8)] = o;
            }
        }
    }
}

}
}
```

### chinesechesszero_b200/net.py

```python
from __future__ import annotations

import os

import numpy as np
import torch
import torch.nn.functional as F
from torch import nn

from . import _lib

PIECES = 7
PLAYS = 17
N_ACTIONS = _lib.N_ACTIONS
FLOP_PER_POSITION = 2 * 4_275_314_716


class ResBlock(nn.Module):

    def __init__(self, num_channels=256):
        super().__init__()
        self.conv1 = nn.Conv2d(num_channels, num_channels, kernel_size=(3, 3), stride=(1, 1), padding=1)
        self.conv1_bn = nn.BatchNorm2d(num_channels)
        self.conv1_act = nn.ReLU()
        self.conv2 = nn.Conv2d(num_channels, num_channels, kernel_size=(3, 3), stride=(1, 1), padding=1)
        self.conv2_bn = nn.BatchNorm2d(num_channels)
        self.conv2_act = nn.ReLU()

    def forward(self, x):
        y = self.conv1_act(self.conv1_bn(self.conv1(x)))
        y = self.conv2_bn(self.conv2(y))
        return self.conv2_act(x + y)


class Net(nn.Module):

    def __init__(self, num_channels=256, resblocks_num=40):
        super().__init__()
        self.input_channels = PLAYS * PIECES
        self.conv_block = nn.Conv2d(self.input_channels, num_channels, kernel_size=(3, 3), stride=(1, 1), padding=1)
        self.conv_block_bn = nn.BatchNorm2d(num_channels)
        self.conv_block_act = nn.ReLU()
        self.res_blocks = nn.ModuleList([ResBlock(num_channels=num_channels) for _ in range(resblocks_num)])
        self.policy_conv = nn.Conv2d(num_channels, PLAYS, kernel_size=(1, 1), stride=(1, 1))
        self.policy_bn = nn.BatchNorm2d(PLAYS)
        self.policy_act = nn.ReLU()
        self.policy_fc = nn.Linear(PLAYS * 10 * 9, N_ACTIONS)
        self.value_conv = nn.Conv2d(num_channels, PIECES, kernel_size=(1, 1), stride=(1, 1))
        self.value_bn = nn.BatchNorm2d(PIECES)
        self.value_act1 = nn.ReLU()
        self.value_fc1 = nn.Linear(PIECES * 10 * 9, 256)
        self.value_act2 = nn.ReLU()
        self.value_fc2 = nn.Linear(256, 1)

    def forward(self, x):
        x = x.view(x.shape[0], -1, 10, 9)
        x = self.conv_block_act(self.conv_block_bn(self.conv_block(x)))
        for block in self.res_blocks:
            x = block(x)
        policy = self.policy_act(self.policy_bn(self.policy_conv(x)))
        policy = self.policy_fc(torch.reshape(policy, [-1, PLAYS * 10 * 9]))
        policy = F.log_softmax(policy, dim=1)
        value = self.value_act1(self.value_bn(self.value_conv(x)))
        value = self.value_act2(self.value_fc1(torch.reshape(value, [-1, PIECES * 10 * 9])))
        value = torch.tanh(self.value_fc2(value))
        return policy, value


def _round_up(n: int, m: int) -> int:
    return (n + m - 1) // m * m


def _fold(conv: nn.Conv2d, bn: nn.BatchNorm2d):
    w = conv.weight.detach().float()
    b = conv.bias.detach().float() if conv.bias is not None else torch.zeros(w.shape[0], device=w.device)
    scale = bn.weight.detach().float() / torch.sqrt(bn.running_var.detach().float() + bn.eps)
    return w * scale.view(-1, 1, 1, 1), (b - bn.running_mean.detach().float()) * scale + bn.bias.detach().float()


def stem_tables(w: torch.Tensor, b: torch.Tensor):
    wf = w.float()
    co = wf.shape[0]
    table = torch.zeros((9, 16, co), dtype=torch.float32, device=w.device)
    for t in range(1, 8):
        table[:, t, :] = wf[:, 7 * PIECES + t - 1].reshape(co, 9).t()
        table[:, 8 + t, :] = wf[:, 15 * PIECES + t - 1].reshape(co, 9).t()
    turn_w = wf[:, 16 * PIECES:17 * PIECES].sum(1)
    bias_turn = torch.zeros((2, 9, co), dtype=torch.float32, device=w.device)
    for rc in range(3):
        for cc in range(3):
            rows = [r for r in range(3) if not (rc == 0 and r == 0) and not (rc == 2 and r == 2)]
            cols = [c for c in range(3) if not (cc == 0 and c == 0) and not (cc == 2 and c == 2)]
            bias_turn[0, rc * 3 + cc] = b.float()
            bias_turn[1, rc * 3 + cc] = b.float() + turn_w[:, rows][:, :, cols].sum((1, 2))
    return table.to(torch.bfloat16).contiguous(), bias_turn.contiguous()


class BatchedEvaluator:

    CONV_IMPLS = ("k9", "k9_skip", "cudnn", "torch")

    def __init__(self, net: Net, device="cuda", dtype=torch.bfloat16, fused_epilogue: bool = True,
                 conv_impl: str | None = None, chunk: int | None = None):
        self.device = torch.device(device)
        self.dtype = dtype
        self.chunk = int(os.environ.get("CCZ_EVAL_CHUNK", "0")) if chunk is None else int(chunk)
        if conv_impl is None:
            conv_impl = os.environ.get("CCZ_CONV_IMPL", "k9") if fused_epilogue else "torch"
        if conv_impl not in self.CONV_IMPLS:
            raise ValueError(f"conv_impl must be one of {self.CONV_IMPLS}")
        k9_ok = self.device.type == "cuda" and dtype == torch.bfloat16 and net.conv_block.out_channels == 256
        if conv_impl in ("k9", "k9_skip") and not k9_ok:
            conv_impl = "cudnn"
        self.conv_impl = conv_impl
        self.fused = conv_impl != "torch"
        self.n_evals = 0
        self.use_heads_pack = os.environ.get("CCZ_HEADS_PACK", "1") != "0"
        self.conv_events: list | None = None
        self.refresh(net)

    def _keep(self, key: str, t: torch.Tensor) -> torch.Tensor:
        old = self._params.get(key)
        if old is not None and old.shape == t.shape and old.dtype == t.dtype and old.stride() == t.stride():
            old.copy_(t)
            return old
        self._params[key] = t
        return t

    @torch.no_grad()
    def refresh(self, net: Net) -> None:
        dev, dt = self.device, self.dtype
        cl = torch.channels_last
        if not hasattr(self, "_params"):
            self._params: dict[str, torch.Tensor] = {}
            self.version = 0
        self.version += 1
        keep = self._keep

        def conv_params(key, conv, bn):
            w, b = _fold(conv, bn)
            return (keep(key + ".w", w.to(dev, dt).contiguous(memory_format=cl)), keep(key + ".b", b.to(dev, dt)),
                    keep(key + ".b32", b.to(dev, torch.float32).contiguous()))

        self.stem = conv_params("stem", net.conv_block, net.conv_block_bn)
        if self.conv_impl in ("k9", "k9_skip"):
            table, bias_turn = stem_tables(self.stem[0], self.stem[2])
            self.stem_lookup = (keep("stem.table", table), keep("stem.bias_turn", bias_turn))
        else:
            self.stem_lookup = None
        self.blocks = [(conv_params(f"rb{i}.1", rb.conv1, rb.conv1_bn), conv_params(f"rb{i}.2", rb.conv2, rb.conv2_bn))
                       for i, rb in enumerate(net.res_blocks)]
        pw, pb = _fold(net.policy_conv, net.policy_bn)
        vw, vb = _fold(net.value_conv, net.value_bn)
        self.heads_w = keep("heads.w", torch.cat([pw, vw], 0).to(dev, dt).contiguous(memory_format=cl))
        self.heads_b = keep("heads.b", torch.cat([pb, vb], 0).to(dev, dt))
        self.policy_fc = (keep("pfc.w", net.policy_fc.weight.detach().to(dev, dt).clone()),
                          keep("pfc.b", net.policy_fc.bias.detach().to(dev, torch.float32).clone()))
        self.value_fc1 = (keep("vfc1.w", net.value_fc1.weight.detach().to(dev, dt).clone()),
                          keep("vfc1.b", net.value_fc1.bias.detach().to(dev, dt).clone()))
        self._kp, self._kv, self._np = _round_up(PLAYS * 90, 8), _round_up(PIECES * 90, 8), _round_up(N_ACTIONS, 8)
        wp = torch.zeros((self._np, self._kp), dtype=dt, device=dev)
        wp[:N_ACTIONS, :PLAYS * 90] = self.policy_fc[0]
        wv = torch.zeros((self.value_fc1[0].shape[0], self._kv), dtype=dt, device=dev)
        wv[:, :PIECES * 90] = self.value_fc1[0]
        self._fc_pad = (keep("pfc.pad", wp), keep("vfc1.pad", wv))
        if not hasattr(self, "_head_buf"):
            self._head_buf = {}
        hw = torch.zeros((32, self.heads_w.shape[1]), dtype=dt, device=dev)
        hw[:PLAYS + PIECES] = self.heads_w.reshape(PLAYS + PIECES, -1)
        hb = torch.zeros((32,), dtype=dt, device=dev)
        hb[:PLAYS + PIECES] = self.heads_b
        self._heads_gemm = (keep("heads.gemm_w", hw), keep("heads.gemm_b", hb))
        self.value_fc2 = (keep("vfc2.w", net.value_fc2.weight.detach().to(dev, torch.float32).clone()),
                          keep("vfc2.b", net.value_fc2.bias.detach().to(dev, torch.float32).clone()))

    def _k9(self, x, w, b32, skip, out):
        if self.conv_events is None:
            return _lib.conv3x3_c256(x, w, b32, skip=skip, out=out)
        e0, e1 = torch.cuda.Event(enable_timing=True), torch.cuda.Event(enable_timing=True)
        e0.record()
        y = _lib.conv3x3_c256(x, w, b32, skip=skip, out=out)
        e1.record()
        self.conv_events.append((skip is not None, e0, e1))
        return y

    def _conv_relu(self, x, wb, k9=False):
        w, b, b32 = wb
        if k9:
            return self._k9(x, w, b32, None, None)
        if self.fused:
            return torch.cudnn_convolution_relu(x, w, b, (1, 1), (1, 1), (1, 1), 1)
        return F.relu_(F.conv2d(x, w, b, padding=1))

    def _conv_add_relu(self, x, wb, skip, k9=False):
        w, b, b32 = wb
        if k9:
            return self._k9(x, w, b32, skip, skip)
        if self.fused:
            return torch.cudnn_convolution_add_relu(x, w, skip, 1.0, b, (1, 1), (1, 1), (1, 1), 1)
        return F.relu_(F.conv2d(x, w, b, padding=1).add_(skip))

    @property
    def needs_planes(self) -> bool:
        return self.stem_lookup is None

    @torch.no_grad()
    def forward(self, planes: torch.Tensor | None, boards: torch.Tensor | None = None):
        use_boards = boards is not None and self.stem_lookup is not None
        g = boards.shape[0] if use_boards else planes.shape[0]
        if self.chunk and g > self.chunk:
            parts = [self._forward(None if use_boards else planes[i:i + self.chunk],
                                   boards[i:i + self.chunk] if use_boards else None) for i in range(0, g, self.chunk)]
            return torch.cat([p[0] for p in parts]), torch.cat([p[1] for p in parts])
        return self._forward(None if use_boards else planes, boards if use_boards else None)

    def _forward(self, planes, boards=None):
        if boards is not None:
            g = boards.shape[0]
            x = _lib.stem_lookup(boards, *self.stem_lookup)
        else:
            g = planes.shape[0]
            x = planes.view(g, PLAYS * PIECES, 10, 9).contiguous(memory_format=torch.channels_last)
            x = self._conv_relu(x, self.stem)
        k9_plain, k9_skip = self.conv_impl == "k9", self.conv_impl in ("k9", "k9_skip")
        for c1, c2 in self.blocks:
            y = self._conv_relu(x, c1, k9_plain)
            x = self._conv_add_relu(y, c2, x, k9_skip)
        if self.device.type == "cuda":
            rows = x.permute(0, 2, 3, 1).reshape(g * 90, x.shape[1])
            h = F.linear(rows, *self._heads_gemm)
            buf = self._head_buf.get(g)
            if buf is None:
                buf = self._head_buf[g] = torch.zeros((g, self._kp + self._kv), dtype=h.dtype, device=h.device)
                if len(self._head_buf) > 8:
                    self._head_buf.pop(next(iter(self._head_buf)))
            if self.dtype == torch.bfloat16 and self.use_heads_pack:
                _lib.heads_pack(h, buf, self._kp)
            else:
                h = F.relu_(h).view(g, 90, 32)
                buf[:, :PLAYS * 90].view(g, PLAYS, 90).copy_(h[:, :, :PLAYS].transpose(1, 2))
                buf[:, self._kp:self._kp + PIECES * 90].view(g, PIECES, 90).copy_(h[:, :, PLAYS:PLAYS + PIECES].transpose(1, 2))
            logits = F.linear(buf[:, :self._kp], self._fc_pad[0])[:, :N_ACTIONS].float() + self.policy_fc[1]
            v = F.relu_(F.linear(buf[:, self._kp:], self._fc_pad[1], self.value_fc1[1])).float()
        else:
            h = F.relu_(F.conv2d(x, self.heads_w, self.heads_b))
            hp = h[:, :PLAYS].reshape(g, PLAYS * 90)
            hv = h[:, PLAYS:].reshape(g, PIECES * 90)
            logits = F.linear(hp, self.policy_fc[0]).float() + self.policy_fc[1]
            v = F.relu_(F.linear(hv, *self.value_fc1)).float()
        v = torch.tanh(F.linear(v, *self.value_fc2)).view(g)
        return logits, v

    def __call__(self, planes, leaf_boards=None):
        logits, v = self.forward(planes, leaf_boards)
        self.n_evals += logits.shape[0]
        return logits, _lib.POLICY_LOGITS, v


class PolicyValueNet:

    def __init__(self, model=None, use_gpu=True, num_channels=256, resblocks_num=40):
        self.use_gpu = use_gpu
        self.l2_const = 2e-3
        self.device = torch.device("cuda") if (use_gpu and torch.cuda.is_available()) else torch.device("cpu")
        self.policy_value_net = Net(num_channels, resblocks_num).to(self.device)
        self.optimizer = torch.optim.Adam(self.policy_value_net.parameters(), lr=1e-3, betas=(0.9, 0.999), eps=1e-8,
                                          weight_decay=self.l2_const)
        if model:
            self.policy_value_net.load_state_dict(torch.load(model, map_location=self.device))
        self._evaluator = None

    def evaluator(self, **kw) -> BatchedEvaluator:
        if self.device.type != "cuda":
            raise _lib.CczError("BatchedEvaluator needs a CUDA device; there is no CPU fallback")
        if self._evaluator is None:
            self.policy_value_net.eval()
            self._evaluator = BatchedEvaluator(self.policy_value_net, self.device, **kw)
        return self._evaluator

    def policy_value(self, state_batch):
        self.policy_value_net.eval()
        if not isinstance(state_batch, torch.Tensor):
            state_batch = torch.tensor(np.asarray(state_batch), dtype=torch.float)
        state_batch = state_batch.to(self.device, torch.float32)
        with torch.no_grad():
            log_act_probs, value = self.policy_value_net(state_batch)
        return np.exp(log_act_probs.cpu().numpy()), value.cpu().numpy()

    def policy_value_fn(self, board, red_states=None, black_states=None):
        rec = board.record() if hasattr(board, "record") else board
        boards = torch.as_tensor(np.ascontiguousarray(rec, dtype=np.uint8).reshape(1, 96)).to(self.device)
        ids, counts, _, planes = _lib.movegen_encode(boards)
        logits, v = self.evaluator().forward(planes)
        probs = torch.softmax(logits, dim=1)[0].cpu().numpy()
        legal = ids[0, : int(counts[0])].cpu().numpy().astype(np.int64)
        return zip(legal.tolist(), probs[legal]), v.cpu().numpy().reshape(1, 1)

    def save_model(self, model_file):
        torch.save(self.policy_value_net.state_dict(), model_file)
```

### include/ccz_b200.h

```cpp
#ifndef CCZ_B200_H
#define CCZ_B200_H

#include <stdint.h>

#ifdef __cplusplus
extern "C" {
#endif

typedef struct CUstream_st *ccz_stream_t;

#define CCZ_BOARD_BYTES 96
#define CCZ_MAX_MOVES 128
#define CCZ_N_ACTIONS 2086
#define CCZ_PLANE_ELEMS 10710
#define CCZ_KEY_WINDOW 128

#define CCZ_FLAG_CHECK 1
#define CCZ_FLAG_NOMOVES 2
#define CCZ_FLAG_INSUFFICIENT 4
#define CCZ_FLAG_FOURFOLD 8
#define CCZ_FLAG_SIXTY 16
#define CCZ_FLAG_TIE_MASK (CCZ_FLAG_INSUFFICIENT | CCZ_FLAG_FOURFOLD | CCZ_FLAG_SIXTY)

#define CCZ_STATUS_EXPAND_FAILED 1
#define CCZ_STATUS_TREE_DROPPED 2
#define CCZ_STATUS_NODE_OVERFLOW CCZ_STATUS_EXPAND_FAILED

#define CCZ_POLICY_PROBS 0
#define CCZ_POLICY_LOGITS 1

#define CCZ_ADVANCE_NEW_GAME (-1)
#define CCZ_ADVANCE_DROP_TREE (-2)
#define CCZ_ADVANCE_KEEP (-3)

typedef struct {
    int32_t visits;
    float value;
    float prior;
    int32_t first_child;
} ccz_node;
typedef struct {
    int32_t parent;
    int16_t move;
    int16_t n_child;
} ccz_link;

#define CCZ_CTL_HEAD 0
#define CCZ_CTL_TAIL 1
#define CCZ_CTL_EXPAND_FAILED 2
#define CCZ_CTL_TREES_DROPPED 3
#define CCZ_CTL_MIN_FREE 4
#define CCZ_CTL_WORDS 8

typedef struct {
    int32_t n_games;
    int32_t n_pages;
    int32_t page_shift;
    int32_t max_pages;
    ccz_node *d_nodes;
    ccz_link *d_links;
    int32_t *d_free_ring;
    int64_t *d_pool_ctl;
    int32_t *d_page_list;
    int32_t *d_page_fill;
    int32_t *d_n_pages;
    int32_t *d_n_pages_new;
    int32_t *d_list_sel;
    int32_t *d_alloc_page;
    int32_t *d_alloc_off;
    int32_t *d_root;
    int32_t *d_n_nodes;
    int32_t *d_status;
    uint8_t *d_root_boards;
    uint64_t *d_root_keys;
} ccz_arena;

int ccz_version(void);
const char *ccz_last_error(void);

int ccz_init(void);

int ccz_action_table(int16_t *id_of, uint8_t *from_of, uint8_t *to_of);

typedef struct {
    uint8_t class_rank[8];
    uint8_t from_descending;
    uint8_t to_descending;
    uint8_t capture_mode;
    uint8_t check_king_first;
} ccz_order_policy;

int ccz_set_order_policy(const ccz_order_policy *p);
int ccz_get_order_policy(ccz_order_policy *out);

int ccz_boards_start(uint8_t *d_boards, int n, ccz_stream_t s);

int ccz_movegen_encode(const uint8_t *d_boards, int n, int16_t *d_move_ids ,
                       int16_t *d_counts , uint8_t *d_flags ,
                       void *d_planes_bf16 , ccz_stream_t s);

int ccz_board_push(uint8_t *d_boards, const int16_t *d_move_ids, int n, uint64_t *d_keys,
                   ccz_stream_t s);

int ccz_board_keys_init(const uint8_t *d_boards, int n, uint64_t *d_keys, ccz_stream_t s);

int ccz_mcts_pool_init(const ccz_arena *a, ccz_stream_t s);

int ccz_mcts_reset(const ccz_arena *a, const uint8_t *d_mask , ccz_stream_t s);

int ccz_mcts_reserve(const ccz_arena *a, int pages_per_game, ccz_stream_t s);

int ccz_mcts_migrate(const ccz_arena *src, const ccz_arena *dst, ccz_stream_t s);

int ccz_mcts_select(const ccz_arena *a, float c_puct, uint8_t *d_leaf_boards ,
                    int32_t *d_leaf_nodes , ccz_stream_t s);

int ccz_mcts_expand_backup(const ccz_arena *a, const int32_t *d_leaf_nodes, const float *d_policy,
                           int policy_kind, const float *d_values ,
                           const int16_t *d_move_ids, const int16_t *d_counts,
                           const uint8_t *d_flags, ccz_stream_t s);

int ccz_mcts_root_visits(const ccz_arena *a, int16_t *d_acts ,
                         int32_t *d_visits , int16_t *d_counts , ccz_stream_t s);

int ccz_mcts_advance(const ccz_arena *a, const int16_t *d_chosen, ccz_stream_t s);

int ccz_replay_pack(const uint8_t *d_hist_boards ,
                    const uint8_t *d_turn_plane , const int16_t *d_acts ,
                    const double *d_probs , const int16_t *d_counts, int n,
                    void *d_states_f16 , double *d_pi , ccz_stream_t s);

int ccz_conv3x3_c256(const void *d_x, const void *d_w, const float *d_bias, const void *d_skip, void *d_y,
                     int n_boards, int variant, ccz_stream_t s);

int ccz_conv3x3_plan(int n_boards, int variant, int resident_clusters, int32_t *out);

int ccz_stem_lookup(const uint8_t *d_boards, int n, const void *d_table, const float *d_bias_turn, void *d_y,
                    ccz_stream_t s);

int ccz_heads_pack(const void *d_h, int n, void *d_operands, int row_elems, int value_off, ccz_stream_t s);

#ifdef __cplusplus
}
#endif
#endif
```

Measured before the change: 378.8.

## Deduplicate leaf boards on device before network eval with device-side counts

Adds a leaf_unique kernel that compacts duplicate leaf boards into a unique set plus a row map. The stem lookup and conv kernels then read the unique count from device memory, so they do no work on the duplicate tail, and heads_pack gathers results back through the row map. This avoids evaluating the network repeatedly on identical positions, such as transpositions or repeated leaves across games, without a host sync. The cost is an extra dedup kernel per eval. Grids are still sized for the full capacity, so early-exiting CTAs remain, and the heads GEMM still runs over all rows.

```diff
diff --git a/chinesechesszero_b200/_lib.py b/chinesechesszero_b200/_lib.py
--- a/chinesechesszero_b200/_lib.py
+++ b/chinesechesszero_b200/_lib.py
@@ -23,6 +23,7 @@
 NODE_BYTES = 24
 MAX_CHILDREN = 119
 POLICY_PROBS, POLICY_LOGITS = 0, 1
+DEDUP_MAX_BOARDS = 16384
 CONV_VARIANT_1CTA, CONV_VARIANT_PAIR, CONV_VARIANT_2PAIRS, CONV_VARIANT_4PAIRS = 1, 2, 2 | 32, 2 | 64
 
 EXPORTS = (
@@ -31,7 +32,7 @@
     "ccz_movegen_encode", "ccz_board_keys_init", "ccz_board_push", "ccz_mcts_pool_init", "ccz_mcts_reset",
     "ccz_mcts_reserve", "ccz_mcts_migrate", "ccz_mcts_select",
     "ccz_mcts_expand_backup", "ccz_mcts_root_visits", "ccz_mcts_advance", "ccz_replay_pack", "ccz_conv3x3_c256", "ccz_conv3x3_plan", "ccz_stem_lookup",
-    "ccz_heads_pack",
+    "ccz_heads_pack", "ccz_conv3x3_c256_count", "ccz_stem_lookup_count", "ccz_heads_pack_rows", "ccz_leaf_unique",
 )
 
 
@@ -113,6 +114,10 @@
     lib.ccz_stem_lookup.argtypes = [vp, i32, vp, vp, vp, vp]
     lib.ccz_conv3x3_plan.argtypes = [i32, i32, i32, vp]
     lib.ccz_heads_pack.argtypes = [vp, i32, vp, i32, i32, vp]
+    lib.ccz_conv3x3_c256_count.argtypes = [vp, vp, vp, vp, vp, i32, vp, i32, vp]
+    lib.ccz_stem_lookup_count.argtypes = [vp, i32, vp, vp, vp, vp, vp]
+    lib.ccz_heads_pack_rows.argtypes = [vp, i32, vp, vp, i32, i32, vp]
+    lib.ccz_leaf_unique.argtypes = [vp, i32, vp, vp, vp, vp, vp]
     for name in EXPORTS:
         if name not in ("ccz_last_error",):
             getattr(lib, name).restype = i32
@@ -364,8 +369,13 @@
     return states, pi
 
 
+def _check_count(count: torch.Tensor, dev) -> None:
+    if count.dtype != torch.int32 or count.numel() != 1 or count.device != dev:
+        raise CczError("count must be a one-element int32 tensor on the boards' device")
+
+
 def conv3x3_c256(x: torch.Tensor, w: torch.Tensor, bias: torch.Tensor, skip: torch.Tensor | None = None,
-                 out: torch.Tensor | None = None, variant: int = 0) -> torch.Tensor:
+                 out: torch.Tensor | None = None, variant: int = 0, count: torch.Tensor | None = None) -> torch.Tensor:
     cl = torch.channels_last
     if x.dtype != torch.bfloat16 or w.dtype != torch.bfloat16 or bias.dtype != torch.float32:
         raise CczError("conv3x3_c256: x and w must be bfloat16, bias float32")
@@ -383,16 +393,20 @@
         raise CczError("conv3x3_c256: variant out of range (see ccz_conv3x3_c256 in include/ccz_b200.h)")
     if not (x.is_cuda and w.is_cuda and bias.is_cuda and out.is_cuda):
         raise CczError("device tensor expected (the C ABI takes device pointers)")
+    sk = None if skip is None else skip.data_ptr()
     with torch.cuda.device(x.device):
-        check(
-            load().ccz_conv3x3_c256(x.data_ptr(), w.data_ptr(), bias.data_ptr(), None if skip is None else skip.data_ptr(),
-                                    out.data_ptr(), int(x.shape[0]), int(variant), stream_ptr(x.device)),
-            "ccz_conv3x3_c256",
-        )
+        if count is None:
+            check(load().ccz_conv3x3_c256(x.data_ptr(), w.data_ptr(), bias.data_ptr(), sk, out.data_ptr(), int(x.shape[0]),
+                                          int(variant), stream_ptr(x.device)), "ccz_conv3x3_c256")
+        else:
+            _check_count(count, x.device)
+            check(load().ccz_conv3x3_c256_count(x.data_ptr(), w.data_ptr(), bias.data_ptr(), sk, out.data_ptr(), int(x.shape[0]),
+                                                count.data_ptr(), int(variant), stream_ptr(x.device)), "ccz_conv3x3_c256_count")
     return out
 
 
-def stem_lookup(boards: torch.Tensor, table: torch.Tensor, bias_turn: torch.Tensor, out: torch.Tensor | None = None) -> torch.Tensor:
+def stem_lookup(boards: torch.Tensor, table: torch.Tensor, bias_turn: torch.Tensor, out: torch.Tensor | None = None,
+                count: torch.Tensor | None = None) -> torch.Tensor:
     n = boards.shape[0]
     if boards.dtype != torch.uint8 or boards.shape[1:] != (BOARD_BYTES,):
         raise CczError("stem_lookup: boards must be uint8 (n,96)")
@@ -404,19 +418,45 @@
     elif tuple(out.shape) != (n, 256, 10, 9) or out.dtype != torch.bfloat16 or not out.is_contiguous(memory_format=torch.channels_last):
         raise CczError("stem_lookup: out must be bf16 (n,256,10,9) channels_last")
     with torch.cuda.device(boards.device):
-        check(load().ccz_stem_lookup(_ptr(boards), n, _ptr(table), _ptr(bias_turn), out.data_ptr(), stream_ptr(boards.device)),
-              "ccz_stem_lookup")
+        if count is None:
+            check(load().ccz_stem_lookup(_ptr(boards), n, _ptr(table), _ptr(bias_turn), out.data_ptr(), stream_ptr(boards.device)),
+                  "ccz_stem_lookup")
+        else:
+            _check_count(count, boards.device)
+            check(load().ccz_stem_lookup_count(_ptr(boards), n, count.data_ptr(), _ptr(table), _ptr(bias_turn), out.data_ptr(),
+                                               stream_ptr(boards.device)), "ccz_stem_lookup_count")
     return out
 
 
-def heads_pack(h: torch.Tensor, operands: torch.Tensor, value_off: int) -> torch.Tensor:
+def heads_pack(h: torch.Tensor, operands: torch.Tensor, value_off: int, rows: torch.Tensor | None = None) -> torch.Tensor:
     n = operands.shape[0]
     if h.dtype != torch.bfloat16 or operands.dtype != torch.bfloat16 or tuple(h.shape) != (n * 90, 32):
         raise CczError("heads_pack: h must be bf16 (n*90, 32) and operands bf16 (n, K)")
     with torch.cuda.device(h.device):
-        check(load().ccz_heads_pack(_ptr(h), n, _ptr(operands), int(operands.shape[1]), int(value_off), stream_ptr(h.device)),
-              "ccz_heads_pack")
+        if rows is None:
+            check(load().ccz_heads_pack(_ptr(h), n, _ptr(operands), int(operands.shape[1]), int(value_off), stream_ptr(h.device)),
+                  "ccz_heads_pack")
+        else:
+            if rows.dtype != torch.int32 or rows.numel() != n:
+                raise CczError("heads_pack: rows must be int32 (n,)")
+            check(load().ccz_heads_pack_rows(_ptr(h), n, _ptr(rows), _ptr(operands), int(operands.shape[1]), int(value_off),
+                                             stream_ptr(h.device)), "ccz_heads_pack_rows")
     return operands
+
+
+def leaf_unique(boards: torch.Tensor, rows: torch.Tensor, uniq: torch.Tensor, n_unique: torch.Tensor,
+                total: torch.Tensor | None = None) -> None:
+    n = boards.shape[0]
+    if boards.dtype != torch.uint8 or boards.shape[1:] != (BOARD_BYTES,) or uniq.dtype != torch.uint8 or uniq.shape != boards.shape:
+        raise CczError("leaf_unique: boards and uniq must be uint8 (n,96)")
+    if rows.dtype != torch.int32 or rows.numel() != n:
+        raise CczError("leaf_unique: rows must be int32 (n,)")
+    _check_count(n_unique, boards.device)
+    if total is not None and (total.dtype != torch.int64 or total.numel() != 1):
+        raise CczError("leaf_unique: total must be int64 (1,)")
+    with torch.cuda.device(boards.device):
+        check(load().ccz_leaf_unique(_ptr(boards), n, _ptr(rows), _ptr(uniq), _ptr(n_unique), _ptr(total),
+                                     stream_ptr(boards.device)), "ccz_leaf_unique")
 
 
 def conv3x3_plan(n_boards: int, variant: int = 0, resident_clusters: int = 74) -> dict:
diff --git a/chinesechesszero_b200/build.py b/chinesechesszero_b200/build.py
--- a/chinesechesszero_b200/build.py
+++ b/chinesechesszero_b200/build.py
@@ -7,7 +7,7 @@
 CSRC = os.path.join(_HERE, "csrc")
 OUT = os.path.join(CSRC, "libccz_b200.so")
 SOURCES = ["ccz_b200.cu"]
-HEADERS = ["ccz_rules.cuh", "ccz_movegen.cuh", "ccz_mcts.cuh", "ccz_replay.cuh", "ccz_conv.cuh", "ccz_stem.cuh", "ccz_heads.cuh", "../../include/ccz_b200.h"]
+HEADERS = ["ccz_rules.cuh", "ccz_movegen.cuh", "ccz_mcts.cuh", "ccz_replay.cuh", "ccz_conv.cuh", "ccz_stem.cuh", "ccz_heads.cuh", "ccz_dedup.cuh", "../../include/ccz_b200.h"]
 NVCC_FLAGS = [
     "-gencode", "arch=compute_100a,code=sm_100a",
     "-lineinfo", "-O3", "-std=c++17",
diff --git a/chinesechesszero_b200/csrc/ccz_b200.cu b/chinesechesszero_b200/csrc/ccz_b200.cu
--- a/chinesechesszero_b200/csrc/ccz_b200.cu
+++ b/chinesechesszero_b200/csrc/ccz_b200.cu
@@ -14,6 +14,7 @@
 #include "ccz_conv.cuh"
 #include "ccz_stem.cuh"
 #include "ccz_heads.cuh"
+#include "ccz_dedup.cuh"
 
 #ifndef CCZ_CONV_DEFAULT_PAIRS
 #define CCZ_CONV_DEFAULT_PAIRS 1
@@ -430,53 +431,123 @@
     return check_launch("replay_pi_kernel");
 }
 
-int ccz_conv3x3_c256(const void *d_x, const void *d_w, const float *d_bias, const void *d_skip, void *d_y, int n_boards,
-                     int variant, ccz_stream_t s) {
+}
+
+namespace {
+
+int conv3x3_c256_impl(const char *name, const void *d_x, const void *d_w, const float *d_bias, const void *d_skip, void *d_y,
+                      int n_boards, const int32_t *d_count, int variant, ccz_stream_t s) {
     namespace cv = ccz::conv;
-    if (n_boards < 0) return fail(-1, "ccz_conv3x3_c256: n_boards < 0");
+    std::string e_name(name);
+    auto bad = [&](int code, const char *what) { return fail(code, (e_name + ": " + what).c_str()); };
+    if (n_boards < 0) return bad(-1, "n_boards < 0");
     if (n_boards == 0) return 0;
-    if (!d_x || !d_w || !d_bias || !d_y) return fail(-1, "ccz_conv3x3_c256: NULL pointer");
-    if (d_y == d_x) return fail(-1, "ccz_conv3x3_c256: output must not alias the input (halo reads)");
-    if (variant < 0 || variant >= 128) return fail(-1, "ccz_conv3x3_c256: bad variant");
+    if (!d_x || !d_w || !d_bias || !d_y) return bad(-1, "NULL pointer");
+    if (d_y == d_x) return bad(-1, "output must not alias the input (halo reads)");
+    if (variant < 0 || variant >= 128) return bad(-1, "bad variant");
     int cta_group = variant & 3;
     const int tail_split = !(variant & 4), dbg = (variant >> 3) & 3;
     int pairs = 1 << ((variant >> 5) & 3);
 #ifndef CCZ_CONV_EXPERIMENTS
-    if (dbg) return fail(-1, "ccz_conv3x3_c256: the load-skipping measurement variants need a -DCCZ_CONV_EXPERIMENTS build");
+    if (dbg) return bad(-1, "the load-skipping measurement variants need a -DCCZ_CONV_EXPERIMENTS build");
 #endif
     if (variant == 0) { cta_group = 2; pairs = CCZ_CONV_DEFAULT_PAIRS; }
     if (cta_group == 0) cta_group = 2;
     if (cta_group == 3 || pairs > 4 || (cta_group == 1 && pairs != 1))
-        return fail(-1, "ccz_conv3x3_c256: unsupported variant (cta_group 1|2, pairs 1|2|4, pairs > 1 needs cta_group 2)");
+        return bad(-1, "unsupported variant (cta_group 1|2, pairs 1|2|4, pairs > 1 needs cta_group 2)");
     if (((uintptr_t)d_x | (uintptr_t)d_w | (uintptr_t)d_y | (uintptr_t)d_skip) & 15)
-        return fail(-1, "ccz_conv3x3_c256: pointers must be 16-byte aligned");
+        return bad(-1, "pointers must be 16-byte aligned");
     static cv::Driver drv;
     if (const char *err = cv::driver_init(drv)) return fail(-3, err);
     const long long m = (long long)n_boards * cv::BOARD_HW;
     const int rows_per_tile = cv::BM * cta_group * pairs;
     const int n_tiles = (int)((m + rows_per_tile - 1) / rows_per_tile);
     CUtensorMap tx, tw, ts, ty;
-    if (!cv::encode_im2col(drv, &tx, d_x, n_boards)) return fail(-3, "ccz_conv3x3_c256: cuTensorMapEncodeIm2col(x) failed");
+    if (!cv::encode_im2col(drv, &tx, d_x, n_boards)) return bad(-3, "cuTensorMapEncodeIm2col(x) failed");
     if (!cv::encode_rows(drv, &tw, d_w, cv::BN, 9 * cv::C, (uint32_t)(cv::BN / cta_group / pairs)))
-        return fail(-3, "ccz_conv3x3_c256: cuTensorMapEncodeTiled(w) failed");
-    if (!cv::encode_rows(drv, &ty, d_y, (uint64_t)m, cv::C, cv::BM)) return fail(-3, "ccz_conv3x3_c256: cuTensorMapEncodeTiled(y) failed");
+        return bad(-3, "cuTensorMapEncodeTiled(w) failed");
+    if (!cv::encode_rows(drv, &ty, d_y, (uint64_t)m, cv::C, cv::BM)) return bad(-3, "cuTensorMapEncodeTiled(y) failed");
     if (d_skip) {
-        if (!cv::encode_rows(drv, &ts, d_skip, (uint64_t)m, cv::C, cv::BM))
-            return fail(-3, "ccz_conv3x3_c256: cuTensorMapEncodeTiled(skip) failed");
+        if (!cv::encode_rows(drv, &ts, d_skip, (uint64_t)m, cv::C, cv::BM)) return bad(-3, "cuTensorMapEncodeTiled(skip) failed");
     } else {
         ts = ty;
     }
     cudaError_t e;
-#define CCZ_CONV_LAUNCH(CG, PAIRS)                                                                                      \
-    (d_skip ? cv::launch_variant<CG, PAIRS, true>(tx, tw, ts, ty, d_bias, n_tiles, tail_split, dbg, s)     \
-            : cv::launch_variant<CG, PAIRS, false>(tx, tw, ts, ty, d_bias, n_tiles, tail_split, dbg, s))
+#define CCZ_CONV_LAUNCH_C(CG, PAIRS, CNT)                                                                                  \
+    (d_skip ? cv::launch_variant<CG, PAIRS, true, CNT>(tx, tw, ts, ty, d_bias, n_tiles, tail_split, dbg, d_count, n_boards, s) \
+            : cv::launch_variant<CG, PAIRS, false, CNT>(tx, tw, ts, ty, d_bias, n_tiles, tail_split, dbg, d_count, n_boards, s))
+#define CCZ_CONV_LAUNCH(CG, PAIRS) (d_count ? CCZ_CONV_LAUNCH_C(CG, PAIRS, true) : CCZ_CONV_LAUNCH_C(CG, PAIRS, false))
     if (cta_group == 1) e = CCZ_CONV_LAUNCH(1, 1);
     else if (pairs == 1) e = CCZ_CONV_LAUNCH(2, 1);
     else if (pairs == 2) e = CCZ_CONV_LAUNCH(2, 2);
     else e = CCZ_CONV_LAUNCH(2, 4);
 #undef CCZ_CONV_LAUNCH
+#undef CCZ_CONV_LAUNCH_C
     if (e != cudaSuccess) return fail(-2, "conv3x3_c256_kernel launch", e);
     return 0;
+}
+
+int stem_lookup_impl(const char *name, const uint8_t *d_boards, int n, const int32_t *d_count, const void *d_table,
+                     const float *d_bias_turn, void *d_y, ccz_stream_t s) {
+    namespace st = ccz::stem;
+    std::string e_name(name);
+    if (n < 0) return fail(-1, (e_name + ": n < 0").c_str());
+    if (n == 0) return 0;
+    if (!d_boards || !d_table || !d_bias_turn || !d_y) return fail(-1, (e_name + ": NULL pointer").c_str());
+    if (((uintptr_t)d_boards & 3) || (((uintptr_t)d_table | (uintptr_t)d_bias_turn | (uintptr_t)d_y) & 15))
+        return fail(-1, (e_name + ": pointers must be 16-byte aligned (boards 4-byte)").c_str());
+    static int n_sm_dev[64] = {0};
+    int dev = 0;
+    CCZ_CUDA(cudaGetDevice(&dev));
+    if (dev < 0 || dev >= 64) return fail(-1, (e_name + ": device index out of range").c_str());
+    int &n_sm = n_sm_dev[dev];
+    if (!n_sm) {
+        CCZ_CUDA(cudaDeviceGetAttribute(&n_sm, cudaDevAttrMultiProcessorCount, dev));
+        CCZ_CUDA(cudaFuncSetAttribute(st::stem_lookup_kernel<false>, cudaFuncAttributeMaxDynamicSharedMemorySize, st::SMEM_BYTES));
+        CCZ_CUDA(cudaFuncSetAttribute(st::stem_lookup_kernel<true>, cudaFuncAttributeMaxDynamicSharedMemorySize, st::SMEM_BYTES));
+    }
+    int blocks = 2 * n_sm;
+    const int need = (n + st::WARPS - 1) / st::WARPS;
+    if (blocks > need) blocks = need;
+    const uint4 *tab = static_cast<const uint4 *>(d_table);
+    const float4 *bt = reinterpret_cast<const float4 *>(d_bias_turn);
+    uint4 *y = static_cast<uint4 *>(d_y);
+    if (d_count)
+        st::stem_lookup_kernel<true><<<blocks, st::WARPS * 32, st::SMEM_BYTES, s>>>(d_boards, n, tab, bt, y, d_count);
+    else
+        st::stem_lookup_kernel<false><<<blocks, st::WARPS * 32, st::SMEM_BYTES, s>>>(d_boards, n, tab, bt, y, nullptr);
+    return check_launch("stem_lookup_kernel");
+}
+
+int heads_pack_impl(const char *name, const void *d_h, int n, const int32_t *d_rows, void *d_operands, int row_elems, int value_off,
+                    ccz_stream_t s) {
+    namespace hd = ccz::heads;
+    std::string e_name(name);
+    if (n < 0) return fail(-1, (e_name + ": n < 0").c_str());
+    if (n == 0) return 0;
+    if (!d_h || !d_operands) return fail(-1, (e_name + ": NULL pointer").c_str());
+    if (((uintptr_t)d_h & 15) || ((uintptr_t)d_operands & 3) || ((uintptr_t)d_rows & 3))
+        return fail(-1, (e_name + ": h must be 16-byte, operands and rows 4-byte aligned").c_str());
+    if ((row_elems & 1) || (value_off & 1) || value_off < hd::N_POLICY * hd::HW || row_elems < value_off + hd::N_VALUE * hd::HW)
+        return fail(-1, (e_name + ": operand row must hold 1530 policy + 630 value elements at even offsets").c_str());
+    hd::heads_pack_kernel<<<n, hd::THREADS, 0, s>>>(static_cast<const uint4 *>(d_h), static_cast<uint32_t *>(d_operands), n,
+                                                  row_elems / 2, value_off / 2, d_rows);
+    return check_launch("heads_pack_kernel");
+}
+
+}
+
+extern "C" {
+
+int ccz_conv3x3_c256(const void *d_x, const void *d_w, const float *d_bias, const void *d_skip, void *d_y, int n_boards,
+                     int variant, ccz_stream_t s) {
+    return conv3x3_c256_impl("ccz_conv3x3_c256", d_x, d_w, d_bias, d_skip, d_y, n_boards, nullptr, variant, s);
+}
+
+int ccz_conv3x3_c256_count(const void *d_x, const void *d_w, const float *d_bias, const void *d_skip, void *d_y, int capacity,
+                           const int32_t *d_n_boards, int variant, ccz_stream_t s) {
+    if (!d_n_boards) return fail(-1, "ccz_conv3x3_c256_count: d_n_boards is NULL");
+    return conv3x3_c256_impl("ccz_conv3x3_c256_count", d_x, d_w, d_bias, d_skip, d_y, capacity, d_n_boards, variant, s);
 }
 
 int ccz_conv3x3_plan(int n_boards, int variant, int resident_clusters, int32_t *out) {
@@ -496,41 +567,46 @@
 }
 
 int ccz_stem_lookup(const uint8_t *d_boards, int n, const void *d_table, const float *d_bias_turn, void *d_y, ccz_stream_t s) {
-    namespace st = ccz::stem;
-    if (n < 0) return fail(-1, "ccz_stem_lookup: n < 0");
-    if (n == 0) return 0;
-    if (!d_boards || !d_table || !d_bias_turn || !d_y) return fail(-1, "ccz_stem_lookup: NULL pointer");
-    if (((uintptr_t)d_boards & 3) || (((uintptr_t)d_table | (uintptr_t)d_bias_turn | (uintptr_t)d_y) & 15))
-        return fail(-1, "ccz_stem_lookup: pointers must be 16-byte aligned (boards 4-byte)");
-    static int n_sm_dev[64] = {0};
+    return stem_lookup_impl("ccz_stem_lookup", d_boards, n, nullptr, d_table, d_bias_turn, d_y, s);
+}
+
+int ccz_stem_lookup_count(const uint8_t *d_boards, int capacity, const int32_t *d_n_boards, const void *d_table, const float *d_bias_turn,
+                          void *d_y, ccz_stream_t s) {
+    if (!d_n_boards) return fail(-1, "ccz_stem_lookup_count: d_n_boards is NULL");
+    return stem_lookup_impl("ccz_stem_lookup_count", d_boards, capacity, d_n_boards, d_table, d_bias_turn, d_y, s);
+}
+
+int ccz_heads_pack(const void *d_h, int n, void *d_operands, int row_elems, int value_off, ccz_stream_t s) {
+    return heads_pack_impl("ccz_heads_pack", d_h, n, nullptr, d_operands, row_elems, value_off, s);
+}
+
+int ccz_heads_pack_rows(const void *d_h, int n, const int32_t *d_rows, void *d_operands, int row_elems, int value_off, ccz_stream_t s) {
+    if (!d_rows) return fail(-1, "ccz_heads_pack_rows: d_rows is NULL");
+    return heads_pack_impl("ccz_heads_pack_rows", d_h, n, d_rows, d_operands, row_elems, value_off, s);
+}
+
+int ccz_leaf_unique(const uint8_t *d_boards, int n, int32_t *d_rows, uint8_t *d_uniq_boards, int32_t *d_n_unique,
+                    unsigned long long *d_unique_total, ccz_stream_t s) {
+    namespace dd = ccz::dedup;
+    if (n < 0 || n > dd::MAX_BOARDS) return fail(-1, "ccz_leaf_unique: n must be 0..16384");
+    if (!d_n_unique) return fail(-1, "ccz_leaf_unique: d_n_unique is NULL");
+    if (n == 0) {
+        CCZ_CUDA(cudaMemsetAsync(d_n_unique, 0, sizeof(int32_t), s));
+        return 0;
+    }
+    if (!d_boards || !d_rows || !d_uniq_boards) return fail(-1, "ccz_leaf_unique: NULL pointer");
+    if (((uintptr_t)d_boards | (uintptr_t)d_uniq_boards) & 15) return fail(-1, "ccz_leaf_unique: boards must be 16-byte aligned");
+    if (d_uniq_boards == d_boards) return fail(-1, "ccz_leaf_unique: uniq_boards must not alias boards");
+    static bool attr_set[64] = {false};
     int dev = 0;
     CCZ_CUDA(cudaGetDevice(&dev));
-    if (dev < 0 || dev >= 64) return fail(-1, "ccz_stem_lookup: device index out of range");
-    int &n_sm = n_sm_dev[dev];
-    if (!n_sm) {
-        CCZ_CUDA(cudaDeviceGetAttribute(&n_sm, cudaDevAttrMultiProcessorCount, dev));
-        CCZ_CUDA(cudaFuncSetAttribute(st::stem_lookup_kernel, cudaFuncAttributeMaxDynamicSharedMemorySize, st::SMEM_BYTES));
-    }
-    int blocks = 2 * n_sm;
-    const int need = (n + st::WARPS - 1) / st::WARPS;
-    if (blocks > need) blocks = need;
-    st::stem_lookup_kernel<<<blocks, st::WARPS * 32, st::SMEM_BYTES, s>>>(d_boards, n, static_cast<const uint4 *>(d_table),
-                                                                         reinterpret_cast<const float4 *>(d_bias_turn),
-                                                                         static_cast<uint4 *>(d_y));
-    return check_launch("stem_lookup_kernel");
-}
-
-int ccz_heads_pack(const void *d_h, int n, void *d_operands, int row_elems, int value_off, ccz_stream_t s) {
-    namespace hd = ccz::heads;
-    if (n < 0) return fail(-1, "ccz_heads_pack: n < 0");
-    if (n == 0) return 0;
-    if (!d_h || !d_operands) return fail(-1, "ccz_heads_pack: NULL pointer");
-    if (((uintptr_t)d_h & 15) || ((uintptr_t)d_operands & 3)) return fail(-1, "ccz_heads_pack: h must be 16-byte, operands 4-byte aligned");
-    if ((row_elems & 1) || (value_off & 1) || value_off < hd::N_POLICY * hd::HW || row_elems < value_off + hd::N_VALUE * hd::HW)
-        return fail(-1, "ccz_heads_pack: operand row must hold 1530 policy + 630 value elements at even offsets");
-    hd::heads_pack_kernel<<<n, hd::THREADS, 0, s>>>(static_cast<const uint4 *>(d_h), static_cast<uint32_t *>(d_operands), n,
-                                                  row_elems / 2, value_off / 2);
-    return check_launch("heads_pack_kernel");
-}
-
-}
+    if (dev < 0 || dev >= 64) return fail(-1, "ccz_leaf_unique: device index out of range");
+    if (!attr_set[dev]) {
+        CCZ_CUDA(cudaFuncSetAttribute(dd::leaf_unique_kernel, cudaFuncAttributeMaxDynamicSharedMemorySize, dd::smem_bytes(dd::MAX_BOARDS)));
+        attr_set[dev] = true;
+    }
+    dd::leaf_unique_kernel<<<1, dd::THREADS, dd::smem_bytes(n), s>>>(d_boards, n, d_rows, d_uniq_boards, d_n_unique, d_unique_total);
+    return check_launch("leaf_unique_kernel");
+}
+
+}
diff --git a/chinesechesszero_b200/csrc/ccz_conv.cuh b/chinesechesszero_b200/csrc/ccz_conv.cuh
--- a/chinesechesszero_b200/csrc/ccz_conv.cuh
+++ b/chinesechesszero_b200/csrc/ccz_conv.cuh
@@ -240,11 +240,28 @@
     return {n_full + (j >> split_log2), (j & ((1 << split_log2) - 1)) * n_w, n_w};
 }
 
-template <int CG, int PAIRS, bool HAS_SKIP>
+struct Plan {
+    int n_items, n_full, split_log2, clusters;
+};
+__host__ __device__ inline Plan plan_items(int n_tiles, int clusters, bool tail_split) {
+    const int rem = n_tiles % clusters;
+    int split_log2 = 0;
+    if (tail_split && rem > 0) {
+        while (split_log2 < 2 && (rem << (split_log2 + 1)) <= clusters) ++split_log2;
+    }
+    Plan p;
+    p.split_log2 = split_log2;
+    p.n_full = split_log2 ? n_tiles - rem : n_tiles;
+    p.n_items = p.n_full + (split_log2 ? rem << split_log2 : 0);
+    p.clusters = clusters > p.n_items ? p.n_items : clusters;
+    return p;
+}
+
+template <int CG, int PAIRS, bool HAS_SKIP, bool DEV_COUNT>
 __global__ void __launch_bounds__(THREADS, 1)
 conv3x3_c256_kernel(const __grid_constant__ CUtensorMap tm_x, const __grid_constant__ CUtensorMap tm_w,
                     const __grid_constant__ CUtensorMap tm_skip, const __grid_constant__ CUtensorMap tm_y, const float *__restrict__ bias,
-                    int n_items, int n_full, int split_log2, int dbg) {
+                    int n_items, int n_full, int split_log2, int dbg, const int32_t *__restrict__ d_count, int count_cap, int tail_split) {
     using K = Cfg<CG>;
     extern __shared__ uint8_t smem_raw[];
     const uint32_t smem_base = (smem_u32(smem_raw) + 1023u) & ~1023u;
@@ -268,6 +285,13 @@
     const uint32_t rank = CLUSTER > 1 ? cluster_ctarank() : 0u;
     const uint32_t prank = rank % CG, pair_id = rank / CG, lead_rank = rank - prank;
     const int cluster_id = blockIdx.x / CLUSTER, n_clusters = gridDim.x / CLUSTER;
+    if constexpr (DEV_COUNT) {
+        const int nb = min(max(*d_count, 0), count_cap), rows_per_tile = BM * CLUSTER;
+        const Plan pl = plan_items((nb * BOARD_HW + rows_per_tile - 1) / rows_per_tile, n_clusters, tail_split != 0);
+        n_items = pl.n_items;
+        n_full = pl.n_full;
+        split_log2 = pl.split_log2;
+    }
 
     if (warp == 0 && lane == 0) {
         tma_prefetch_desc(&tm_x);
@@ -488,27 +512,10 @@
                     CU_TENSOR_MAP_FLOAT_OOB_FILL_NONE) == CUDA_SUCCESS;
 }
 
-struct Plan {
-    int n_items, n_full, split_log2, clusters;
-};
-inline Plan plan_items(int n_tiles, int clusters, bool tail_split) {
-    const int rem = n_tiles % clusters;
-    int split_log2 = 0;
-    if (tail_split && rem > 0) {
-        while (split_log2 < 2 && (rem << (split_log2 + 1)) <= clusters) ++split_log2;
-    }
-    Plan p;
-    p.split_log2 = split_log2;
-    p.n_full = split_log2 ? n_tiles - rem : n_tiles;
-    p.n_items = p.n_full + (split_log2 ? rem << split_log2 : 0);
-    p.clusters = clusters > p.n_items ? p.n_items : clusters;
-    return p;
-}
-
-template <int CG, int PAIRS, bool HAS_SKIP>
+template <int CG, int PAIRS, bool HAS_SKIP, bool DEV_COUNT>
 inline cudaError_t launch_variant(const CUtensorMap &tx, const CUtensorMap &tw, const CUtensorMap &ts, const CUtensorMap &ty, const float *bias,
-                                  int n_tiles, int tail_split, int dbg, cudaStream_t stream) {
-    auto kern = conv3x3_c256_kernel<CG, PAIRS, HAS_SKIP>;
+                                  int n_tiles, int tail_split, int dbg, const int32_t *d_count, int count_cap, cudaStream_t stream) {
+    auto kern = conv3x3_c256_kernel<CG, PAIRS, HAS_SKIP, DEV_COUNT>;
     constexpr int CLUSTER = CG * PAIRS;
     static int max_clusters_dev[64] = {0};
     int dev = 0, n_sm = 0;
@@ -539,10 +546,14 @@
         if (n < 1) return cudaErrorInvalidConfiguration;
         max_clusters = n < n_sm / CLUSTER ? n : n_sm / CLUSTER;
     }
+    if constexpr (DEV_COUNT) {
+        cfg.gridDim = dim3((unsigned)(max_clusters * CLUSTER));
+        return cudaLaunchKernelEx(&cfg, kern, tx, tw, ts, ty, bias, 0, 0, 0, dbg, d_count, count_cap, tail_split);
+    }
     const Plan pl = plan_items(n_tiles, max_clusters, tail_split != 0);
     cfg.gridDim = dim3((unsigned)(pl.clusters * CLUSTER));
-    return cudaLaunchKernelEx(&cfg, kern, tx, tw, ts, ty, bias, pl.n_items, pl.n_full, pl.split_log2, dbg);
-}
-
-}
-}
+    return cudaLaunchKernelEx(&cfg, kern, tx, tw, ts, ty, bias, pl.n_items, pl.n_full, pl.split_log2, dbg, (const int32_t *)nullptr, 0, 0);
+}
+
+}
+}
diff --git a/chinesechesszero_b200/csrc/ccz_dedup.cuh b/chinesechesszero_b200/csrc/ccz_dedup.cuh
--- /dev/null
+++ b/chinesechesszero_b200/csrc/ccz_dedup.cuh
@@ -0,0 +1,111 @@
+#pragma once
+
+#include <cuda_runtime.h>
+
+#include <cstdint>
+
+namespace ccz {
+namespace dedup {
+
+constexpr int THREADS = 1024;
+constexpr int MAX_BOARDS = 16384;
+constexpr int KEY_WORDS = 23;
+constexpr uint32_t EMPTY = 0x7fffffffu;
+
+__host__ __device__ inline int table_slots(int n) {
+    int t = 64;
+    while (t < 2 * n) t <<= 1;
+    return t;
+}
+__host__ __device__ inline int smem_bytes(int n) { return (table_slots(n) + n) * 4; }
+
+__device__ __forceinline__ uint32_t key_word(const uint32_t *rec, int i) { return i < KEY_WORDS - 1 ? rec[i] : rec[i] & 0x00FFFFFFu; }
+
+__global__ void __launch_bounds__(THREADS, 1)
+leaf_unique_kernel(const uint8_t *__restrict__ boards, int n, int32_t *__restrict__ rows, uint8_t *__restrict__ uniq,
+                   int32_t *__restrict__ n_unique, unsigned long long *__restrict__ total) {
+    extern __shared__ uint32_t sm[];
+    const int T = table_slots(n);
+    uint32_t *table = sm;
+    int32_t *rep = (int32_t *)(sm + T);
+    __shared__ int warp_sum[THREADS / 32];
+    for (int i = threadIdx.x; i < T; i += THREADS) table[i] = EMPTY;
+    __syncthreads();
+
+    for (int g = threadIdx.x; g < n; g += THREADS) {
+        const uint32_t *rec = reinterpret_cast<const uint32_t *>(boards + (size_t)g * 96);
+        uint32_t key[KEY_WORDS];
+        uint64_t h = 0x9E3779B97F4A7C15ull;
+#pragma unroll
+        for (int i = 0; i < KEY_WORDS; ++i) {
+            key[i] = key_word(rec, i);
+            h = (h ^ key[i]) * 0x100000001B3ull;
+            h ^= h >> 29;
+        }
+        h *= 0xBF58476D1CE4E5B9ull;
+        int slot = (int)((h ^ (h >> 32)) & (uint64_t)(T - 1));
+        for (;;) {
+            uint32_t v = atomicCAS(&table[slot], EMPTY, (uint32_t)g);
+            if (v == EMPTY) break;
+            const uint32_t *other = reinterpret_cast<const uint32_t *>(boards + (size_t)v * 96);
+            bool same = true;
+#pragma unroll
+            for (int i = 0; i < KEY_WORDS; ++i) same &= key_word(other, i) == key[i];
+            if (same) {
+                atomicMin(&table[slot], (uint32_t)g);
+                break;
+            }
+            slot = (slot + 1) & (T - 1);
+        }
+        rep[g] = slot;
+    }
+    __syncthreads();
+    for (int g = threadIdx.x; g < n; g += THREADS) rep[g] = (int32_t)table[rep[g]];
+    __syncthreads();
+
+    const int per = (n + THREADS - 1) / THREADS, lo = threadIdx.x * per, hi = min(lo + per, n);
+    int cnt = 0;
+    for (int g = lo; g < hi; ++g) cnt += rep[g] == g;
+    const int lane = threadIdx.x & 31, warp = threadIdx.x >> 5;
+    int incl = cnt;
+#pragma unroll
+    for (int d = 1; d < 32; d <<= 1) {
+        const int y = __shfl_up_sync(0xffffffffu, incl, d);
+        if (lane >= d) incl += y;
+    }
+    if (lane == 31) warp_sum[warp] = incl;
+    __syncthreads();
+    if (warp == 0) {
+        int s = warp_sum[lane];
+#pragma unroll
+        for (int d = 1; d < 32; d <<= 1) {
+            const int y = __shfl_up_sync(0xffffffffu, s, d);
+            if (lane >= d) s += y;
+        }
+        warp_sum[lane] = s;
+    }
+    __syncthreads();
+    int next = incl - cnt + (warp ? warp_sum[warp - 1] : 0);
+    for (int g = lo; g < hi; ++g)
+        if (rep[g] == g) table[g] = (uint32_t)next++;
+    if (threadIdx.x == 0) {
+        const int u = warp_sum[THREADS / 32 - 1];
+        *n_unique = u;
+        if (total) atomicAdd(total, (unsigned long long)u);
+    }
+    __syncthreads();
+
+    for (int g = threadIdx.x; g < n; g += THREADS) {
+        const int r = (int)table[rep[g]];
+        rows[g] = r;
+        if (rep[g] == g) {
+            const uint4 *src = reinterpret_cast<const uint4 *>(boards + (size_t)g * 96);
+            uint4 *dst = reinterpret_cast<uint4 *>(uniq + (size_t)r * 96);
+#pragma unroll
+            for (int i = 0; i < 6; ++i) dst[i] = src[i];
+        }
+    }
+}
+
+}
+}
diff --git a/chinesechesszero_b200/csrc/ccz_heads.cuh b/chinesechesszero_b200/csrc/ccz_heads.cuh
--- a/chinesechesszero_b200/csrc/ccz_heads.cuh
+++ b/chinesechesszero_b200/csrc/ccz_heads.cuh
@@ -9,11 +9,11 @@
 
 __global__ void __launch_bounds__(THREADS)
 heads_pack_kernel(const uint4 *__restrict__ h , uint32_t *__restrict__ out , int n,
-                  int row_words, int value_word_off) {
+                  int row_words, int value_word_off, const int32_t *__restrict__ rows) {
     __shared__ __align__(16) uint16_t s_t[HW][CH + 2];
     const int b = blockIdx.x;
     if (b >= n) return;
-    const uint4 *src = h + (size_t)b * (HW * CH * 2 / 16);
+    const uint4 *src = h + (size_t)(rows ? rows[b] : b) * (HW * CH * 2 / 16);
     for (int i = threadIdx.x; i < HW * CH * 2 / 16; i += THREADS) {
         const uint4 v = src[i];
         const int row = i >> 2, col = (i & 3) * 8;
diff --git a/chinesechesszero_b200/csrc/ccz_stem.cuh b/chinesechesszero_b200/csrc/ccz_stem.cuh
--- a/chinesechesszero_b200/csrc/ccz_stem.cuh
+++ b/chinesechesszero_b200/csrc/ccz_stem.cuh
@@ -23,9 +23,11 @@
     }
 }
 
+template <bool DEV_COUNT>
 __global__ void __launch_bounds__(WARPS * 32, 2)
 stem_lookup_kernel(const uint8_t *__restrict__ boards, int n, const uint4 *__restrict__ table, const float4 *__restrict__ bias_turn,
-                   uint4 *__restrict__ y) {
+                   uint4 *__restrict__ y, const int32_t *__restrict__ d_count) {
+    if constexpr (DEV_COUNT) n = min(*d_count, n);
     extern __shared__ __align__(16) uint8_t smem[];
     uint4 *tab_s = reinterpret_cast<uint4 *>(smem);
     float4 *bt_s = reinterpret_cast<float4 *>(smem + TABLE_ELEMS * 2);
diff --git a/chinesechesszero_b200/net.py b/chinesechesszero_b200/net.py
--- a/chinesechesszero_b200/net.py
+++ b/chinesechesszero_b200/net.py
@@ -100,7 +100,7 @@
     CONV_IMPLS = ("k9", "k9_skip", "cudnn", "torch")
 
     def __init__(self, net: Net, device="cuda", dtype=torch.bfloat16, fused_epilogue: bool = True,
-                 conv_impl: str | None = None, chunk: int | None = None):
+                 conv_impl: str | None = None, chunk: int | None = None, dedup: bool = True):
         self.device = torch.device(device)
         self.dtype = dtype
         self.chunk = int(os.environ.get("CCZ_EVAL_CHUNK", "0")) if chunk is None else int(chunk)
@@ -113,7 +113,11 @@
             conv_impl = "cudnn"
         self.conv_impl = conv_impl
         self.fused = conv_impl != "torch"
+        self.dedup = bool(dedup)
         self.n_evals = 0
+        self._n_unique_host = 0
+        self._unique_total = torch.zeros(1, dtype=torch.int64, device=self.device) if self.device.type == "cuda" else None
+        self._dedup_buf: dict = {}
         self.use_heads_pack = os.environ.get("CCZ_HEADS_PACK", "1") != "0"
         self.conv_events: list | None = None
         self.refresh(net)
@@ -173,28 +177,28 @@
         self.value_fc2 = (keep("vfc2.w", net.value_fc2.weight.detach().to(dev, torch.float32).clone()),
                           keep("vfc2.b", net.value_fc2.bias.detach().to(dev, torch.float32).clone()))
 
-    def _k9(self, x, w, b32, skip, out):
+    def _k9(self, x, w, b32, skip, out, count=None):
         if self.conv_events is None:
-            return _lib.conv3x3_c256(x, w, b32, skip=skip, out=out)
+            return _lib.conv3x3_c256(x, w, b32, skip=skip, out=out, count=count)
         e0, e1 = torch.cuda.Event(enable_timing=True), torch.cuda.Event(enable_timing=True)
         e0.record()
-        y = _lib.conv3x3_c256(x, w, b32, skip=skip, out=out)
+        y = _lib.conv3x3_c256(x, w, b32, skip=skip, out=out, count=count)
         e1.record()
         self.conv_events.append((skip is not None, e0, e1))
         return y
 
-    def _conv_relu(self, x, wb, k9=False):
+    def _conv_relu(self, x, wb, k9=False, count=None):
         w, b, b32 = wb
         if k9:
-            return self._k9(x, w, b32, None, None)
+            return self._k9(x, w, b32, None, None, count)
         if self.fused:
             return torch.cudnn_convolution_relu(x, w, b, (1, 1), (1, 1), (1, 1), 1)
         return F.relu_(F.conv2d(x, w, b, padding=1))
 
-    def _conv_add_relu(self, x, wb, skip, k9=False):
+    def _conv_add_relu(self, x, wb, skip, k9=False, count=None):
         w, b, b32 = wb
         if k9:
-            return self._k9(x, w, b32, skip, skip)
+            return self._k9(x, w, b32, skip, skip, count)
         if self.fused:
             return torch.cudnn_convolution_add_relu(x, w, skip, 1.0, b, (1, 1), (1, 1), (1, 1), 1)
         return F.relu_(F.conv2d(x, w, b, padding=1).add_(skip))
@@ -213,18 +217,41 @@
             return torch.cat([p[0] for p in parts]), torch.cat([p[1] for p in parts])
         return self._forward(None if use_boards else planes, boards if use_boards else None)
 
+    @property
+    def n_unique(self) -> int:
+        dev = int(self._unique_total.item()) if self._unique_total is not None else 0
+        return self._n_unique_host + dev
+
+    def _dedup_buffers(self, g: int):
+        buf = self._dedup_buf.get(g)
+        if buf is None:
+            z = dict(device=self.device)
+            buf = self._dedup_buf[g] = (torch.zeros(g, dtype=torch.int32, **z), torch.zeros((g, _lib.BOARD_BYTES), dtype=torch.uint8, **z),
+                                        torch.zeros(1, dtype=torch.int32, **z))
+            if len(self._dedup_buf) > 8:
+                self._dedup_buf.pop(next(iter(self._dedup_buf)))
+        return buf
+
     def _forward(self, planes, boards=None):
+        row_map = count = None
         if boards is not None:
             g = boards.shape[0]
-            x = _lib.stem_lookup(boards, *self.stem_lookup)
+            if self.dedup and self.conv_impl == "k9" and g <= _lib.DEDUP_MAX_BOARDS:
+                row_map, uniq, count = self._dedup_buffers(g)
+                _lib.leaf_unique(boards, row_map, uniq, count, self._unique_total)
+                boards = uniq
+            else:
+                self._n_unique_host += g
+            x = _lib.stem_lookup(boards, *self.stem_lookup, count=count)
         else:
             g = planes.shape[0]
             x = planes.view(g, PLAYS * PIECES, 10, 9).contiguous(memory_format=torch.channels_last)
             x = self._conv_relu(x, self.stem)
+            self._n_unique_host += g
         k9_plain, k9_skip = self.conv_impl == "k9", self.conv_impl in ("k9", "k9_skip")
         for c1, c2 in self.blocks:
-            y = self._conv_relu(x, c1, k9_plain)
-            x = self._conv_add_relu(y, c2, x, k9_skip)
+            y = self._conv_relu(x, c1, k9_plain, count)
+            x = self._conv_add_relu(y, c2, x, k9_skip, count)
         if self.device.type == "cuda":
             rows = x.permute(0, 2, 3, 1).reshape(g * 90, x.shape[1])
             h = F.linear(rows, *self._heads_gemm)
@@ -234,9 +261,11 @@
                 if len(self._head_buf) > 8:
                     self._head_buf.pop(next(iter(self._head_buf)))
             if self.dtype == torch.bfloat16 and self.use_heads_pack:
-                _lib.heads_pack(h, buf, self._kp)
+                _lib.heads_pack(h, buf, self._kp, rows=row_map)
             else:
                 h = F.relu_(h).view(g, 90, 32)
+                if row_map is not None:
+                    h = h.index_select(0, row_map)
                 buf[:, :PLAYS * 90].view(g, PLAYS, 90).copy_(h[:, :, :PLAYS].transpose(1, 2))
                 buf[:, self._kp:self._kp + PIECES * 90].view(g, PIECES, 90).copy_(h[:, :, PLAYS:PLAYS + PIECES].transpose(1, 2))
             logits = F.linear(buf[:, :self._kp], self._fc_pad[0])[:, :N_ACTIONS].float() + self.policy_fc[1]
diff --git a/include/ccz_b200.h b/include/ccz_b200.h
--- a/include/ccz_b200.h
+++ b/include/ccz_b200.h
@@ -133,12 +133,24 @@
 int ccz_conv3x3_c256(const void *d_x, const void *d_w, const float *d_bias, const void *d_skip, void *d_y,
                      int n_boards, int variant, ccz_stream_t s);
 
+int ccz_conv3x3_c256_count(const void *d_x, const void *d_w, const float *d_bias, const void *d_skip, void *d_y,
+                           int capacity, const int32_t *d_n_boards, int variant, ccz_stream_t s);
+
 int ccz_conv3x3_plan(int n_boards, int variant, int resident_clusters, int32_t *out);
 
 int ccz_stem_lookup(const uint8_t *d_boards, int n, const void *d_table, const float *d_bias_turn, void *d_y,
                     ccz_stream_t s);
 
+int ccz_stem_lookup_count(const uint8_t *d_boards, int capacity, const int32_t *d_n_boards, const void *d_table,
+                          const float *d_bias_turn, void *d_y, ccz_stream_t s);
+
 int ccz_heads_pack(const void *d_h, int n, void *d_operands, int row_elems, int value_off, ccz_stream_t s);
+
+int ccz_heads_pack_rows(const void *d_h, int n, const int32_t *d_rows, void *d_operands, int row_elems, int value_off,
+                        ccz_stream_t s);
+
+int ccz_leaf_unique(const uint8_t *d_boards, int n, int32_t *d_rows, uint8_t *d_uniq_boards, int32_t *d_n_unique,
+                    unsigned long long *d_unique_total, ccz_stream_t s);
 
 #ifdef __cplusplus
 }
```

Measured after the change: 411.0, median of 6. +8.5%, better.
